# galatolofederico/clip-glass

Hardware: AMD Instinct MI355X
Metric: candidate latents scored/sec (GAN→CLIP fitness), StyleGAN2_ffhq_d pop=64 (higher is better)
Workload: dtype f16; 1 GPU; StyleGAN2_ffhq_d: StyleGAN2 config-f 1024px G+D + CLIP ViT-B/32, pop=64 per GPU, batch_size=4, n_obj=2; pop_per_gpu=64, global_pop=64, batch_size=4, parallelism=population-shard x1, device=AMD Radeon Graphics (gfx950:sramecc+:xnack-), 256 CUs, hbm_gib=288

## Files before the change

### clip_glass_amd/csrc/clip.cpp

```cpp
#include <math.h>
#include <string.h>

#include "engine.h"

extern "C" int glass_clip_geometry_supported(int32_t width, int32_t layers, int32_t heads, int32_t patch, int32_t res, int32_t embed) {
    char msg[256];
#define GEOM_REQ(cond, ...)                       \
    if (!(cond)) {                                \
        snprintf(msg, sizeof msg, __VA_ARGS__);   \
        glass_set_error(msg);                     \
        return GLASS_ERR_ARG;                     \
    }
    GEOM_REQ(width > 0 && layers > 0 && heads > 0 && patch > 0 && res > 0 && embed > 0,
             "unsupported CLIP geometry: width, layers, heads, patch, resolution and embed must be positive");
    GEOM_REQ(width % heads == 0 && width / heads == 64,
             "unsupported CLIP geometry: head dim must be 64 (width %d / heads %d)", width, heads);
    GEOM_REQ(res % patch == 0, "unsupported CLIP geometry: resolution %d is not a multiple of patch %d", res, patch);
    GEOM_REQ(patch <= 64 && res / patch <= 63,
             "unsupported CLIP geometry: patch %d / grid %d out of range (patch <= 64, at most 63 x 63 patches)", patch, res / patch);
    GEOM_REQ(layers <= 64 && width <= 4096 && embed <= 4096, "unsupported CLIP geometry: layers %d / width %d / embed %d out of range",
             layers, width, embed);
#undef GEOM_REQ
    return GLASS_OK;
}
int clip_patch_k(const glass_config& c) { return (3 * c.clip_patch * c.clip_patch + 63) / 64 * 64; }

extern "C" int glass_clip_preprocess_supported(int32_t gen_res, int32_t clip_res, int32_t clip_resize, int32_t clip_normalize) {
    if (clip_resize < 0 || clip_resize > 2) {
        glass_set_error("clip_resize must be 0 (point-sampled bilinear: the reference), 1 (antialiased bilinear) or 2 (antialiased bicubic), got " +
                        std::to_string(clip_resize));
        return GLASS_ERR_ARG;
    }
    if (clip_normalize < 0 || clip_normalize > 1) {
        glass_set_error("clip_normalize must be 0 (none: the reference) or 1 (CLIP mean / std), got " + std::to_string(clip_normalize));
        return GLASS_ERR_ARG;
    }
    if (clip_resize == 0 || gen_res == 0) return GLASS_OK;
    ResizeTaps t;
    std::string why;
    if (!build_resize_taps(gen_res, clip_res, clip_resize, t, why)) {
        glass_set_error(why);
        return GLASS_ERR_ARG;
    }
    return GLASS_OK;
}

static int load_clip_blocks(glass_engine* e, const char* prefix, int layers, int W, std::vector<ClipBlock>& out) {
    char nm[256];
    int rc;
    for (int i = 0; i < layers; ++i) {
        snprintf(nm, sizeof nm, "%s%d.", prefix, i);
        const std::string p = nm;
        ClipBlock b;
        GET(l1g, p + "ln_1.weight");
        GET(l1b, p + "ln_1.bias");
        GET(l2g, p + "ln_2.weight");
        GET(l2b, p + "ln_2.bias");
        GET(wq, p + "attn.in_proj_weight");
        GET(bq, p + "attn.in_proj_bias");
        GET(wo, p + "attn.out_proj.weight");
        GET(bo, p + "attn.out_proj.bias");
        GET(wf, p + "mlp.c_fc.weight");
        GET(bf, p + "mlp.c_fc.bias");
        GET(wp, p + "mlp.c_proj.weight");
        GET(bp, p + "mlp.c_proj.bias");
        REQUIRE(numel(wq) == (size_t)3 * W * W && numel(wo) == (size_t)W * W && numel(wf) == (size_t)4 * W * W &&
                    numel(wp) == (size_t)4 * W * W,
                GLASS_ERR_ARG, "bad CLIP block shapes: " + p);
        if ((rc = upload(e, &b.ln1_g, l1g->data))) return rc;
        if ((rc = upload(e, &b.ln1_b, l1b->data))) return rc;
        if ((rc = upload(e, &b.ln2_g, l2g->data))) return rc;
        if ((rc = upload(e, &b.ln2_b, l2b->data))) return rc;
        if ((rc = upload(e, &b.w_qkv, to_half(wq->data.data(), numel(wq))))) return rc;
        if ((rc = upload(e, &b.w_out, to_half(wo->data.data(), numel(wo))))) return rc;
        if ((rc = upload(e, &b.w_fc, to_half(wf->data.data(), numel(wf))))) return rc;
        if ((rc = upload(e, &b.w_proj, to_half(wp->data.data(), numel(wp))))) return rc;
        if ((rc = upload(e, &b.b_qkv, bq->data))) return rc;
        if ((rc = upload(e, &b.b_out, bo->data))) return rc;
        if ((rc = upload(e, &b.b_fc, bf->data))) return rc;
        if ((rc = upload(e, &b.b_proj, bp->data))) return rc;
        out.push_back(b);
    }
    return GLASS_OK;
}

int finalize_clip(glass_engine* e) {
    const glass_config& c = e->cfg;
    const int W = c.clip_width, ps = c.clip_patch, G = c.clip_res / ps, T = G * G + 1, E = c.clip_embed;
    const std::string v = "clip.visual.";
    GET(conv1, v + "conv1.weight");
    GET(cls, v + "class_embedding");
    GET(pos, v + "positional_embedding");
    GET(lg, v + "ln_pre.weight");
    GET(lb, v + "ln_pre.bias");
    GET(pg, v + "ln_post.weight");
    GET(pb, v + "ln_post.bias");
    GET(proj, v + "proj");
    REQUIRE(numel(conv1) == (size_t)W * 3 * ps * ps && numel(cls) == (size_t)W && numel(pos) == (size_t)T * W &&
                numel(proj) == (size_t)W * E,
            GLASS_ERR_ARG, "bad CLIP visual shapes");
    const int K = 3 * ps * ps, Kp = clip_patch_k(c);
    std::vector<_Float16> pw = to_half(conv1->data.data(), numel(conv1));
    if (Kp != K) {
        std::vector<_Float16> padded((size_t)W * Kp, (_Float16)0.f);
        for (int n = 0; n < W; ++n) std::copy(pw.begin() + (size_t)n * K, pw.begin() + (size_t)(n + 1) * K, padded.begin() + (size_t)n * Kp);
        pw.swap(padded);
    }
    int rc = upload(e, &e->c_patch_w, pw);
    if (rc) return rc;
    if ((rc = upload(e, &e->c_cls, cls->data))) return rc;
    if ((rc = upload(e, &e->c_pos, pos->data))) return rc;
    if ((rc = upload(e, &e->c_lnpre_g, lg->data))) return rc;
    if ((rc = upload(e, &e->c_lnpre_b, lb->data))) return rc;
    if ((rc = upload(e, &e->c_lnpost_g, pg->data))) return rc;
    if ((rc = upload(e, &e->c_lnpost_b, pb->data))) return rc;
    if ((rc = upload(e, &e->c_proj, proj->data))) return rc;
    int rc2 = load_clip_blocks(e, "clip.visual.transformer.resblocks.", c.clip_layers, W, e->cblk);
    if (rc2) return rc2;
    if (find(e, "clip.token_embedding.weight") != nullptr) {
        GET(tok, "clip.token_embedding.weight");
        GET(tpos, "clip.positional_embedding");
        GET(fg, "clip.ln_final.weight");
        GET(fb, "clip.ln_final.bias");
        GET(tp, "clip.text_projection");
        REQUIRE(tok->dims.size() == 2 && tpos->dims.size() == 2 && tpos->dims[1] == tok->dims[1], GLASS_ERR_ARG,
                "bad CLIP text embedding shapes");
        e->t_vocab = (int)tok->dims[0];
        e->t_width = (int)tok->dims[1];
        e->t_ctx = (int)tpos->dims[0];
        REQUIRE(e->t_width % 64 == 0 && numel(tp) == (size_t)e->t_width * E, GLASS_ERR_ARG, "bad CLIP text projection shape");
        int nl = 0;
        char nm2[256];
        for (;; ++nl) {
            snprintf(nm2, sizeof nm2, "clip.transformer.resblocks.%d.ln_1.weight", nl);
            if (!find(e, nm2)) break;
        }
        if ((rc = upload(e, &e->t_tok, tok->data))) return rc;
        if ((rc = upload(e, &e->t_pos, tpos->data))) return rc;
        if ((rc = upload(e, &e->t_lnf_g, fg->data))) return rc;
        if ((rc = upload(e, &e->t_lnf_b, fb->data))) return rc;
        if ((rc = upload(e, &e->t_proj, tp->data))) return rc;
        if ((rc = load_clip_blocks(e, "clip.transformer.resblocks.", nl, e->t_width, e->tblk))) return rc;
    }
    return GLASS_OK;
}

int finalize_preprocess(glass_engine* e) {
    const glass_config& c = e->cfg;
    if (c.clip_resize == 0 || e->R == 0) return GLASS_OK;
    ResizeTaps t;
    std::string why;
    REQUIRE(build_resize_taps(e->R, c.clip_res, c.clip_resize, t, why), GLASS_ERR_ARG, why);
    float* d_table = nullptr;
    int rc = upload(e, &d_table, t.table);
    if (rc) return rc;
    e->rz.table = d_table; e->rz.n4 = (int)(t.table.size() / 4); e->rz.ts = t.ts; e->rz.lds_bytes = t.lds_bytes;
    return GLASS_OK;
}

static void run_blocks(glass_engine* e, const std::vector<ClipBlock>& blk, int l0, int l1, float* x, half_t* ln16, half_t* qkv, half_t* att,
                       half_t* hid, int T, int seqs, int W, int heads, int causal, hipStream_t st, const char* pfx) {
    const int M = seqs * T;
    char buf[48];
    auto tag = [&](const char* op) -> const char* {
        if (!pfx) return nullptr;
        snprintf(buf, sizeof buf, "%s.%s", pfx, op);
        return buf;
    };
    auto gemm = [&](const GemmParams& g, const char* op) {
        if (pfx) run_gemm(e, g, tag(op));
        else if (!launch_gemm_tiled(g, st)) launch_gemm_direct(g, st);
    };
    auto layernorm = [&](const float* g, const float* b) {
        Prof pr(e, tag("layernorm"), 0, 6.0 * M * W);
        launch_layernorm(x, W, M, W, g, b, ln16, nullptr, st);
    };
    for (int li = l0; li < l1; ++li) {
        const ClipBlock& b = blk[li];
        layernorm(b.ln1_g, b.ln1_b);
        gemm(gemm_params(ln16, b.w_qkv, M, 3 * W, W, b.b_qkv, 0, qkv, nullptr, T), "qkv");
        {
            Prof pr(e, tag("attention"), 4.0 * seqs * heads * (double)T * T * 64, 8.0 * M * W);
            launch_attention(qkv, seqs, T, heads, 64, causal, att, st);
        }
        gemm(gemm_params(att, b.w_out, M, W, W, b.b_out, 2, nullptr, x, T), "attn_out");
        layernorm(b.ln2_g, b.ln2_b);
        gemm(gemm_params(ln16, b.w_fc, M, 4 * W, W, b.b_fc, 1, hid, nullptr, T), "mlp_fc");
        gemm(gemm_params(hid, b.w_proj, M, W, 4 * W, b.b_proj, 2, nullptr, x, T), "mlp_proj");
    }
}

void run_clip_embed(glass_engine* e, int P) {
    const glass_config& c = e->cfg;
    const int W = c.clip_width, G = c.clip_res / c.clip_patch, T = G * G + 1;
    run_gemm(e, gemm_params(e->d_patches, e->c_patch_w, P * G * G, W, clip_patch_k(c), nullptr, 3, nullptr, e->d_pe, G * G), "clip.patch_embed");
    Prof pr(e, "clip.embed_lnpre", 0, 8.0 * P * T * W);
    launch_embed_lnpre(e->d_pe, e->c_cls, e->c_pos, e->c_lnpre_g, e->c_lnpre_b, P, T, W, e->d_x, e->cur);
}
void run_clip_layers(glass_engine* e, int P, int l0, int l1) {
    const glass_config& c = e->cfg;
    const int G = c.clip_res / c.clip_patch;
    run_blocks(e, e->cblk, l0, std::min(l1, (int)e->cblk.size()), e->d_x, e->d_ln16, e->d_qkv, e->d_attn, e->d_hid, G * G + 1, P, c.clip_width, c.clip_heads, 0, e->cur, "clip");
}
void run_clip_head(glass_engine* e, int P) {
    const glass_config& c = e->cfg;
    const int W = c.clip_width, G = c.clip_res / c.clip_patch, T = G * G + 1;
    Prof pr(e, "clip.head", 2.0 * P * W * c.clip_embed, 4.0 * W * c.clip_embed);
    launch_layernorm(e->d_x, (long long)T * W, P, W, e->c_lnpost_g, e->c_lnpost_b, nullptr, e->d_cls, e->cur);
    launch_dense(e->d_cls, W, P, W, e->c_proj, c.clip_embed, nullptr, e->d_feat, c.clip_embed, 0, 0, nullptr, 0,
                 e->cur);
    launch_cosine(e->d_feat, e->d_target, P, c.clip_embed, e->d_sim, e->cur);
}
void run_clip(glass_engine* e, int P) {
    run_clip_embed(e, P);
    run_clip_layers(e, P, 0, (int)e->cblk.size());
    run_clip_head(e, P);
}

double clip_resize_bytes(const glass_engine* e, int B) {
    const glass_config& c = e->cfg;
    const double out = 2.0 * 3 * c.clip_res * c.clip_res;
    return B * ((c.clip_resize ? 4.0 * 3 * e->R * e->R : 16.0 * c.clip_res * c.clip_res * 3) + out);
}
void run_clip_resize(glass_engine* e, const float* y, int B, half_t* patches) {
    const glass_config& c = e->cfg;
    if (c.clip_resize == 0 && c.clip_normalize == 0)
        launch_resize_patches(y, B, e->R, c.clip_res, c.clip_patch, clip_patch_k(c), patches, e->cur);
    else
        launch_preprocess_patches(y, B, e->R, c.clip_res, c.clip_patch, clip_patch_k(c), c.clip_resize, c.clip_normalize, e->rz, patches, e->cur);
}

void text_work_free(glass_engine* e) {
    for (void* p : e->twork.owned) hipFree(p);
    e->twork = glass_engine::TextWork();
}

extern "C" int glass_engine_encode_text(glass_engine* e, const int32_t* tokens, int32_t n_texts, int32_t ctx, float* out_feat) {
    REQUIRE(e && tokens && out_feat && n_texts > 0, GLASS_ERR_ARG, "null argument");
    REQUIRE(e->finalized, GLASS_ERR_STATE, "finalize() first");
    REQUIRE(e->t_tok != nullptr, GLASS_ERR_STATE, "CLIP text tower weights were not loaded (clip.token_embedding.weight ...)");
    REQUIRE(ctx == e->t_ctx && ctx <= 128, GLASS_ERR_ARG, "context length does not match positional_embedding");
    GLASS_HIP(hipSetDevice(e->cfg.device));
    const int W = e->t_width, heads = W / 64, M = n_texts * ctx, E = e->cfg.clip_embed;
    std::vector<int> eot(n_texts);
    for (int n = 0; n < n_texts; ++n) {
        int best = 0;
        for (int t = 0; t < ctx; ++t) {
            const int v = tokens[(size_t)n * ctx + t];
            REQUIRE(v >= 0 && v < e->t_vocab, GLASS_ERR_ARG, "token id out of range");
            if (v > tokens[(size_t)n * ctx + best]) best = t;
        }
        eot[n] = best;
    }
    auto& tw = e->twork;
    hipError_t err = hipSuccess;
    if (tw.n_texts != n_texts) {
        text_work_free(e);
        if (err == hipSuccess) err = owned_alloc(tw.owned, &tw.d_tok, (size_t)M);
        if (err == hipSuccess) err = owned_alloc(tw.owned, &tw.d_rows, (size_t)n_texts);
        if (err == hipSuccess) err = owned_alloc(tw.owned, &tw.x, (size_t)M * W);
        if (err == hipSuccess) err = owned_alloc(tw.owned, &tw.cls, (size_t)n_texts * W);
        if (err == hipSuccess) err = owned_alloc(tw.owned, &tw.feat, (size_t)n_texts * E);
        if (err == hipSuccess) err = owned_alloc(tw.owned, &tw.ln16, (size_t)M * W);
        if (err == hipSuccess) err = owned_alloc(tw.owned, &tw.qkv, (size_t)M * 3 * W);
        if (err == hipSuccess) err = owned_alloc(tw.owned, &tw.att, (size_t)M * W);
        if (err == hipSuccess) err = owned_alloc(tw.owned, &tw.hid, (size_t)M * 4 * W);
        if (err != hipSuccess) {
            text_work_free(e);
            glass_set_error(std::string("encode_text: hipMalloc failed: ") + hipGetErrorString(err));
            return GLASS_ERR_NOMEM;
        }
        tw.n_texts = n_texts;
    }
    for (int n = 0; n < n_texts; ++n) eot[n] += n * ctx;
    hipStream_t st = e->stream;
    hipMemcpyAsync(tw.d_tok, tokens, (size_t)M * sizeof(int), hipMemcpyHostToDevice, st);
    hipMemcpyAsync(tw.d_rows, eot.data(), (size_t)n_texts * sizeof(int), hipMemcpyHostToDevice, st);
    launch_embed_text(tw.d_tok, e->t_tok, e->t_pos, M, ctx, W, tw.x, st);
    run_blocks(e, e->tblk, 0, (int)e->tblk.size(), tw.x, tw.ln16, tw.qkv, tw.att, tw.hid, ctx, n_texts, W, heads, 1, st, nullptr);
    launch_layernorm_rows(tw.x, tw.d_rows, n_texts, W, e->t_lnf_g, e->t_lnf_b, tw.cls, st);
    launch_dense(tw.cls, W, n_texts, W, e->t_proj, E, nullptr, tw.feat, E, 0, 0, nullptr, 0, st);
    err = hipMemcpyAsync(out_feat, tw.feat, (size_t)n_texts * E * sizeof(float), hipMemcpyDeviceToHost, st);
    if (err == hipSuccess) err = hipStreamSynchronize(st);
    if (err == hipSuccess) err = hipGetLastError();
    if (err != hipSuccess) {
        text_work_free(e);
        glass_set_error(std::string("encode_text failed: ") + hipGetErrorString(err));
        return GLASS_ERR_HIP;
    }
    return GLASS_OK;
}

extern "C" int glass_engine_encode_image(glass_engine* e, const float* images, int32_t n, float* out_feat) {
    REQUIRE(e && images && out_feat && n > 0, GLASS_ERR_ARG, "null argument");
    REQUIRE(e->finalized, GLASS_ERR_STATE, "finalize() first");
    REQUIRE(n <= e->cfg.max_pop, GLASS_ERR_ARG, "more images than max_pop");
    const glass_config& c = e->cfg;
    GLASS_HIP(hipSetDevice(c.device));
    const size_t elems = (size_t)n * 3 * c.clip_res * c.clip_res;
    float* d_img = nullptr;
    GLASS_HIP(hipMalloc(&d_img, elems * sizeof(float)));
    hipError_t err = hipMemcpyAsync(d_img, images, elems * sizeof(float), hipMemcpyHostToDevice, e->stream);
    e->cur = e->stream;
    launch_image_patches(d_img, n, c.clip_res, c.clip_patch, clip_patch_k(c), e->d_patches, e->stream);
    run_clip(e, n);
    if (err == hipSuccess)
        err = hipMemcpyAsync(out_feat, e->d_feat, (size_t)n * c.clip_embed * sizeof(float), hipMemcpyDeviceToHost, e->stream);
    if (err == hipSuccess) err = hipStreamSynchronize(e->stream);
    if (err == hipSuccess) err = hipGetLastError();
    hipFree(d_img);
    e->prof_events.clear();
    e->event_next = 0;
    if (err != hipSuccess) {
        glass_set_error(std::string("encode_image failed: ") + hipGetErrorString(err));
        return GLASS_ERR_HIP;
    }
    return GLASS_OK;
}
```

### clip_glass_amd/csrc/common.h

```cpp
#pragma once
#include <hip/hip_runtime.h>
#include <stdint.h>

#include <atomic>
#include <mutex>
#include <stdio.h>
#include <stdlib.h>

typedef _Float16 half_t;
typedef _Float16 h2 __attribute__((ext_vector_type(2)));
typedef _Float16 h4 __attribute__((ext_vector_type(4)));
typedef _Float16 h8 __attribute__((ext_vector_type(8)));
typedef float f4 __attribute__((ext_vector_type(4)));
typedef float f16x __attribute__((ext_vector_type(16)));

#define GLASS_SQRT2 1.41421356237309504880f

__device__ __forceinline__ f16x mfma32(h8 a, h8 b, f16x c) {
    return __builtin_amdgcn_mfma_f32_32x32x16_f16(a, b, c, 0, 0, 0);
}
__device__ __forceinline__ int mfma32_row(int reg, int lane) { return (reg & 3) + 8 * (reg >> 2) + 4 * (lane >> 5); }
__device__ __forceinline__ void philox4x32_10(uint32_t c[4], uint32_t k0, uint32_t k1) {
#pragma unroll
    for (int i = 0; i < 10; ++i) {
// ... 18 lines not shown
    const int my = oy >> 1, mx = ox >> 1;
    const float wy0 = (oy & 1) ? 0.25f : 0.75f, wx0 = (ox & 1) ? 0.25f : 0.75f;
    float s = 0.f;
    s += ((my >= 1 && mx >= 1) ? wy0 * wx0 : 0.f) * t[0];
    s += (my >= 1 ? wy0 * (1.f - wx0) : 0.f) * t[1];
    s += (mx >= 1 ? (1.f - wy0) * wx0 : 0.f) * t[2];
    s += (1.f - wy0) * (1.f - wx0) * t[3];
    return s;
}

struct DevOnce {
    std::atomic<bool> done[32] = {};
    static int dev() {
        int d = 0;
        if (hipGetDevice(&d) != hipSuccess || d < 0 || d >= 32) return -1;
        return d;
    }
    bool first() const {
        const int d = dev();
        return d < 0 || !done[d].load(std::memory_order_acquire);
    }
    void set() {
        const int d = dev();
        if (d >= 0) done[d].store(true, std::memory_order_release);
    }
    template <class F> void run(F&& setup) {
        if (first()) {
            setup();
            set();
        }
    }
};
struct GlassDevProps { int cus, lds_optin; };
inline GlassDevProps glass_dev_props() {
    static std::atomic<int> cus[32] = {}, lds[32] = {};
    int d = 0;
    if (hipGetDevice(&d) != hipSuccess || d < 0 || d >= 32) d = 0;
    if (!cus[d].load()) {
        hipDeviceProp_t prop;
        if (hipGetDeviceProperties(&prop, d) == hipSuccess) {
            lds[d].store((int)prop.sharedMemPerBlockOptin > 0 ? (int)prop.sharedMemPerBlockOptin : (int)prop.sharedMemPerBlock);
            cus[d].store(prop.multiProcessorCount);
        }
    }
    return GlassDevProps{cus[d].load() > 0 ? cus[d].load() : 256, lds[d].load() > 0 ? lds[d].load() : 64 * 1024};
}
inline int glass_cu_count() { return glass_dev_props().cus; }
inline bool glass_lds_fits(int bytes) {
    const GlassDevProps dp = glass_dev_props();
    if (bytes <= dp.lds_optin) return true;
    static std::mutex mu;
    static int seen_dev[16], seen_bytes[16], n_seen = 0;
    int d = 0;
    (void)hipGetDevice(&d);
    std::lock_guard<std::mutex> lk(mu);
    for (int i = 0; i < n_seen; ++i)
        if (seen_dev[i] == d && seen_bytes[i] == bytes) return false;
    if (n_seen == 16) return false;
    seen_dev[n_seen] = d;
    seen_bytes[n_seen++] = bytes;
    if (n_seen == 16) fprintf(stderr, "libglass: further LDS refusals are not reported\n");
    fprintf(stderr, "libglass: device %d offers %d B of opt-in LDS per workgroup; a kernel family that needs %d B is refused and its "
                    "layers fall back to a slower kernel (expected on gfx950: 163840 B)\n", d, dp.lds_optin, bytes);
    return false;
}

#define GLASS_NOMINAL_POP 64

__device__ __forceinline__ float lrelu_sqrt2(float v) { return (v > 0.f ? v : 0.2f * v) * GLASS_SQRT2; }
struct ActK { float k1, k2; };
__device__ __forceinline__ ActK act_consts(int act, float s) {
    return ActK{(act == 1 ? GLASS_SQRT2 : 1.f) * s, (act == 1 ? 0.2f * GLASS_SQRT2 : act == 2 ? 0.f : 1.f) * s};
}
__device__ __forceinline__ f4 act_apply(f4 v, ActK k) { return __builtin_elementwise_max(v * k.k1, v * k.k2); }

struct ConvParams {
    const half_t* x;
    long long x_bstride;
    int B, H, W, Cin;
    int Hc, Wc;
    int KS, stride, pad;
    const half_t* w;
    const half_t* w_up;
    long long w_bstride;
    int Neff, Cout;
    int up;
    int Ho, Wo;
    const float* sn;
    int sn_stride;
    const half_t* sn16;
    const half_t* pre_shift16;
    const float* pre_shift;
    int in_up;
    const float* dscale;
    int ds_stride;
    const float* noise;
    float noise_strength;
    int batch_size;
    const float* bias;
    const float* shift;
    int act;
    const half_t* res;
    int res_cs;
    int res_up;
    float out_scale;
    const float* rgb_y;
    const float* rgb_w;
    const float* rgb_b;
    half_t* rgb_x_out;
    half_t* rgb_xs_out;
    const float* trgb_w;
    const float* trgb_b;
    const float* trgb_sn;
    int trgb_sn_stride;
    const float* trgb_smax;
    int trgb_smax_stride;
    const float* trgb_yprev;
    float* trgb_yout;
    float* rgb_tanh_out;
    float* trgb_part;
    const half_t* trgb_tab;
    half_t* xs_out;
    const half_t* post_scale16;
    int post_stride;
    const half_t* skip_x;
    const half_t* skip_w;
    int dry_run;
    int x_planar32;
    int x_planar8;
    int y_planar8;
    int row_walk;
    half_t* y;
    float* y32;
};

struct GemmParams {
    const half_t* a;
    const half_t* w;
    int M, N, K;
    const float* bias;
    int mode;
    half_t* out16;
    float* out32;
    int ldo;
    int kpt;
    long long w_tap_stride;
    int batch;
    long long a_bs, w_bs, o_bs;
    int cand_rows;
    int cand_batch;
    int g_on, g_h, g_w, g_hc, g_wc, g_stride, g_pad, g_ks, g_cin;
    long long g_xbs;
    int ld;
};
```

### clip_glass_amd/csrc/engine.cpp

```cpp
#include "engine.h"

#include <math.h>
#include <string.h>

#include <stdlib.h>

static thread_local std::string g_err;
void glass_set_error(const std::string& s) { g_err = s; }
extern "C" const char* glass_last_error(void) { return g_err.c_str(); }
extern "C" const char* glass_version(void) { return "clip-glass-amd 0.1 (gfx950)"; }

void glass_pack_conv(const float* W, int cout, int cin, int ks, int cin_pad, std::vector<_Float16>& out) {
    const float coef = 1.0f / sqrtf((float)cin * ks * ks);
    out.assign((size_t)ks * ks * cout * cin_pad, (_Float16)0.f);
    for (int o = 0; o < cout; ++o)
        for (int i = 0; i < cin; ++i)
            for (int t = 0; t < ks * ks; ++t)
                out[((size_t)t * cout + o) * cin_pad + i] = (_Float16)(W[((size_t)o * cin + i) * ks * ks + t] * coef);
}

int glass_fold_upconv(const float* W, int cout, int cin, std::vector<_Float16>& out) {
    const float coef = 1.0f / sqrtf((float)cin * 9.f);
    const float f1[4] = {1.f, 3.f, 3.f, 1.f};
    float F[4][4];
// ... 324 lines not shown
        DBlock d;
        d.cin = chD(i);
        d.cout = chD(i + 1);
        d.res = e->R >> i;
        snprintf(nm, sizeof nm, "D.conv_blocks.%d", i);
        const std::string p = nm;
        GET(W0, p + ".conv_block.0.layer.weight");
        GET(B0, p + ".conv_block.0.bias");
        GET(W1, p + ".conv_block.1.layer.weight");
        GET(B1, p + ".conv_block.1.bias");
        GET(WS, p + ".projection.weight");
        REQUIRE(numel(W0) == (size_t)d.cin * d.cin * 9 && numel(W1) == (size_t)d.cout * d.cin * 9 &&
                    numel(WS) == (size_t)d.cout * d.cin && numel(B0) == (size_t)d.cin && numel(B1) == (size_t)d.cout,
                GLASS_ERR_ARG, "bad D block shape: " + p);
        std::vector<_Float16> pk;
        glass_pack_conv(W0->data.data(), d.cin, d.cin, 3, d.cin, pk);
        int rc = upload(e, &d.w0, pk);
        if (rc) return rc;
        glass_pack_conv(W1->data.data(), d.cout, d.cin, 3, d.cin, pk);
        rc = upload(e, &d.w1, pk);
        if (rc) return rc;
        glass_pack_conv(WS->data.data(), d.cout, d.cin, 1, d.cin, pk);
        rc = upload(e, &d.wskip, pk);
        if (rc) return rc;
        rc = upload(e, &d.b0, B0->data);
        if (rc) return rc;
        rc = upload(e, &d.b1, B1->data);
        if (rc) return rc;
        e->dblk.push_back(d);
    }
    const int CL = chD(n - 1);
    snprintf(nm, sizeof nm, "D.conv_blocks.%d.1.conv_block.0", n - 1);
    const std::string p = nm;
    GET(WF, p + ".layer.weight");
    GET(BF, p + ".bias");
    REQUIRE(numel(WF) == (size_t)CL * (CL + 1) * 9 && numel(BF) == (size_t)CL, GLASS_ERR_ARG, "bad D final conv shape");
    e->d_final_cpad = ((CL + 1 + 15) / 16) * 16;
    std::vector<_Float16> pk;
    glass_pack_conv(WF->data.data(), CL, CL + 1, 3, e->d_final_cpad, pk);
    int rc = upload(e, &e->d_final_w, pk);
    if (rc) return rc;
    rc = upload(e, &e->d_final_b, BF->data);
    if (rc) return rc;
    GET(W0, "D.dense.0.layer.weight");
    GET(B0, "D.dense.0.bias");
    GET(W1, "D.dense.1.layer.weight");
    GET(B1, "D.dense.1.bias");
    REQUIRE(numel(W0) == (size_t)CL * CL * 16 && numel(B0) == (size_t)CL && numel(W1) == (size_t)CL && numel(B1) == 1,
            GLASS_ERR_ARG, "bad D dense shape");
    std::vector<_Float16> d0((size_t)CL * CL * 16);
    const float coef0 = 1.0f / sqrtf((float)CL * 16.f);
    for (int o = 0; o < CL; ++o)
        for (int ch = 0; ch < CL; ++ch)
            for (int px = 0; px < 16; ++px)
                d0[(size_t)o * CL * 16 + (size_t)px * CL + ch] = (_Float16)(W0->data[(size_t)o * CL * 16 + ch * 16 + px] * coef0);
    rc = upload(e, &e->d_dense0_w, d0);
    if (rc) return rc;
    rc = upload(e, &e->d_dense0_b, B0->data);
    if (rc) return rc;
    rc = upload(e, &e->d_dense1_wt, transposed(W1->data.data(), 1, CL, 1.0f / sqrtf((float)CL)));
    if (rc) return rc;
    return upload(e, &e->d_dense1_b, B1->data);
}

static int alloc_buffers(glass_engine* e) {
    const glass_config& c = e->cfg;
    const int P = c.max_pop, L = c.latent_size, CH = e->chunk;
    int rc;
    if ((rc = dev_alloc(e, &e->d_z, (size_t)P * L))) return rc;
    if ((rc = dev_alloc(e, &e->d_w0, (size_t)P * L))) return rc;
    if ((rc = dev_alloc(e, &e->d_w1, (size_t)P * L))) return rc;
    if ((rc = dev_alloc(e, &e->d_s, (size_t)P * e->S_total))) return rc;
    if ((rc = dev_alloc(e, &e->d_s16, (size_t)P * e->S_total))) return rc;
    if ((rc = dev_alloc(e, &e->d_smax, (size_t)P * e->n_style))) return rc;
    if ((rc = dev_alloc(e, &e->d_trgb_tab, (size_t)P * 32 * 512))) return rc;
    {
        size_t part = 0;
        for (int b = 0; b < c.n_blocks; ++b)
            if (c.channels[b] > 128 && c.channels[b] % 128 == 0 && c.channels[b] <= 512)
                part = std::max(part, (size_t)(c.channels[b] / 128) * (size_t)P * 3 * ((size_t)4 << b) * ((size_t)4 << b));
        if (part && (rc = dev_alloc(e, &e->d_trgb_part, part))) return rc;
    }
    if (e->cfg.generator != GLASS_GEN_BIGGAN_DEEP && e->cfg.n_blocks > 0) {
        int cmax = 16;
        for (int i = 0; i < e->cfg.n_blocks; ++i) cmax = std::max(cmax, (int)e->cfg.channels[i]);
        e->cap_a = 256LL * 9 * cmax;
        e->cap_c = 256LL * 4 * cmax;
        if ((rc = dev_alloc(e, &e->ws_a, (size_t)(e->cap_a * P)))) return rc;
        if ((rc = dev_alloc(e, &e->ws_c, (size_t)(e->cap_c * P)))) return rc;
        if (e->cfg.use_discriminator) {
            if ((rc = dev_alloc(e, &e->ws_a2, (size_t)(e->cap_a * P)))) return rc;
            if ((rc = dev_alloc(e, &e->ws_c2, (size_t)(e->cap_c * P)))) return rc;
        }
    } else if (e->cfg.generator == GLASS_GEN_BIGGAN_DEEP) {
        const int cmax = 4 * e->cfg.bg_ch;
        e->cap_a = 256LL * 9 * cmax;
        e->cap_c = 256LL * 4 * cmax;
        if ((rc = dev_alloc(e, &e->ws_a, (size_t)(e->cap_a * P)))) return rc;
        if ((rc = dev_alloc(e, &e->ws_c, (size_t)(e->cap_c * P)))) return rc;
    }
    if ((rc = dev_alloc(e, &e->d_epsrow, (size_t)P * e->n_style))) return rc;
    if ((rc = dev_alloc(e, &e->d_dscale, (size_t)P * e->D_total))) return rc;
    for (auto& g : e->gconv) {
        const bool fused_ok = g.up && g.cin % 32 == 0 && g.cout % 32 == 0 && g.res_in >= 16;
        const bool tiled_ok = !g.up && g.cin % 32 == 0 && g.cout % 32 == 0 && g.res_in % 32 == 0;
        g.welems = 9LL * g.cin * g.cout;
        g.premod = (fused_ok || tiled_ok) && g.welems * 2 <= (500LL << 10);
        if (g.premod && (rc = dev_alloc(e, &g.wm, (size_t)P * g.welems))) return rc;
    }
    if (c.noise_mode != 0) {
        const int n_mb = P / c.batch_size;
        for (auto& g : e->gconv) {
            float* p;
            if ((rc = dev_alloc(e, &p, (size_t)n_mb * g.res_out * g.res_out))) return rc;
            e->d_noise.push_back(p);
        }
    }
    size_t maxact = 0;
    for (int b = 0; b < c.n_blocks; ++b) {
        const size_t res = 4u << b;
        size_t ch = c.channels[b];
        if (b > 0) ch = std::max<size_t>(ch, c.channels[b - 1]);
        maxact = std::max(maxact, (res + 1) * (res + 1) * ch);
    }
    if (c.n_blocks > 0) maxact = std::max(maxact, (size_t)16 * (c.channels[0] + 16));
    e->act_elems = maxact * CH;
    for (int i = 0; i < 8 && c.n_blocks > 0; ++i)
        if (i >= 6 || c.use_discriminator)
            if ((rc = dev_alloc(e, &e->act[i], e->act_elems))) return rc;
    for (int i = 0; i < 4; ++i)
        if ((rc = dev_alloc(e, &e->ybuf[i], (size_t)CH * 3 * e->R * e->R))) return rc;
    if (c.n_blocks > 0) {
        e->n_low = 0;
        while (e->n_low < c.n_blocks && (4 << e->n_low) <= e->low_res) ++e->n_low;
        if (e->n_low < 1) e->n_low = 1;
        const size_t rl = 4u << (e->n_low - 1);
        size_t cmax = 16;
        for (int b = 0; b < e->n_low; ++b) cmax = std::max<size_t>(cmax, c.channels[b]);
        if (e->n_low < c.n_blocks) cmax = std::max<size_t>(cmax, c.channels[e->n_low]);
        const size_t low_elems = (size_t)P * (rl + 1) * (rl + 1) * (cmax + 16);
        const int n_lowbuf = c.use_discriminator ? 6 : 2;
        for (int i = 0; i < n_lowbuf; ++i)
            if ((rc = dev_alloc(e, &e->low[i], low_elems))) return rc;
        for (int i = 0; i < 2; ++i)
            if ((rc = dev_alloc(e, &e->ylow[i], (size_t)P * 3 * rl * rl))) return rc;
    }
    if ((rc = dev_alloc(e, &e->d_img, (size_t)CH * 3 * e->R * e->R))) return rc;
    const int W = c.clip_width, ps = c.clip_patch, G = c.clip_res / ps, T = G * G + 1;
    const size_t Kp = (size_t)clip_patch_k(c);
    if ((rc = dev_alloc(e, &e->d_patches, (size_t)P * G * G * Kp))) return rc;
    if (Kp != (size_t)3 * ps * ps) GLASS_HIP(hipMemset(e->d_patches, 0, (size_t)P * G * G * Kp * sizeof(half_t)));
    if ((rc = dev_alloc(e, &e->d_pe, (size_t)P * G * G * W))) return rc;
    if ((rc = dev_alloc(e, &e->d_x, (size_t)P * T * W))) return rc;
    if ((rc = dev_alloc(e, &e->d_ln16, (size_t)P * T * W))) return rc;
    if ((rc = dev_alloc(e, &e->d_qkv, (size_t)P * T * 3 * W))) return rc;
    if ((rc = dev_alloc(e, &e->d_attn, (size_t)P * T * W))) return rc;
    if ((rc = dev_alloc(e, &e->d_hid, (size_t)P * T * 4 * W))) return rc;
    if ((rc = dev_alloc(e, &e->d_cls, (size_t)P * W))) return rc;
    if ((rc = dev_alloc(e, &e->d_feat, (size_t)P * c.clip_embed))) return rc;
    if ((rc = dev_alloc(e, &e->d_sim, (size_t)P))) return rc;
    if ((rc = dev_alloc(e, &e->d_dis, (size_t)P))) return rc;
    if ((rc = dev_alloc(e, &e->d_F, (size_t)P * 2))) return rc;
    if ((rc = dev_alloc(e, &e->d_target, (size_t)c.clip_embed))) return rc;
    if (c.use_discriminator && c.n_blocks > 0) {
        if ((rc = dev_alloc(e, &e->d_dfin, (size_t)P * 16 * c.channels[0]))) return rc;
        if ((rc = dev_alloc(e, &e->d_dh, (size_t)P * c.channels[0]))) return rc;
        if ((rc = dev_alloc(e, &e->d_dh_part, (size_t)16 * P * c.channels[0]))) return rc;
    }
    {
        std::vector<DenseDesc> dd;
        for (auto& g : e->gconv) {
            DenseDesc q;
            q.x = e->d_s + g.style_off; q.ldx = e->S_total; q.K = g.cin; q.wt = g.wsq; q.N = g.cout; q.bias = nullptr;
            q.out = e->d_dscale + g.ds_off; q.ldo = e->D_total; q.eps_row = e->d_epsrow + g.style_idx; q.eps_stride = e->n_style;
            dd.push_back(q);
            e->demod_max_n = std::max(e->demod_max_n, g.cout);
        }
        DenseDesc* dptr = nullptr;
        if ((rc = upload(e, &dptr, dd))) return rc;
        e->d_demod_desc = dptr;
    }
    GLASS_HIP(hipMemset(e->d_dis, 0, (size_t)P * sizeof(float)));
    e->h_pinned_bytes = std::max((size_t)P * L, (size_t)P * (c.clip_embed + 8)) * sizeof(float);
    GLASS_HIP(hipHostMalloc((void**)&e->h_pinned, e->h_pinned_bytes, hipHostMallocDefault));
    return GLASS_OK;
}

extern "C" int glass_engine_finalize(glass_engine* e) {
    REQUIRE(e, GLASS_ERR_ARG, "null engine");
    REQUIRE(!e->finalized, GLASS_ERR_STATE, "engine already finalized");
    GLASS_HIP(hipSetDevice(e->cfg.device));
    int rc = GLASS_OK;
    if (e->cfg.n_blocks > 0) {
        if ((rc = finalize_generator(e))) return rc;
        if (e->cfg.use_discriminator && (rc = finalize_discriminator(e))) return rc;
    }
    if (e->cfg.generator == GLASS_GEN_BIGGAN_DEEP && (rc = glass_biggan_finalize(e))) return rc;
    if ((rc = finalize_gpt2(e))) return rc;
    if ((rc = finalize_clip(e))) return rc;
    if ((rc = finalize_preprocess(e))) return rc;
    if ((rc = alloc_buffers(e))) return rc;
    e->host.clear();
    e->finalized = true;
    return GLASS_OK;
}

extern "C" int glass_engine_set_target(glass_engine* e, const float* feat, int32_t n) {
    REQUIRE(e && feat, GLASS_ERR_ARG, "null argument");
    REQUIRE(e->finalized, GLASS_ERR_STATE, "finalize() first");
    REQUIRE(n == e->cfg.clip_embed, GLASS_ERR_ARG, "target feature length != clip_embed");
    GLASS_HIP(hipSetDevice(e->cfg.device));
    GLASS_HIP(hipMemcpy(e->d_target, feat, (size_t)n * sizeof(float), hipMemcpyHostToDevice));
    e->has_target = true;
    return GLASS_OK;
}

void collect_profile(glass_engine* e) {
    std::map<std::string, glass_prof_row> rows;
    std::vector<std::string> order;
    for (auto& pe : e->prof_events) {
        float ms = 0.f;
        hipEventElapsedTime(&ms, pe.e0, pe.e1);
        auto it = rows.find(pe.name);
        if (it == rows.end()) {
            glass_prof_row r;
            memset(&r, 0, sizeof r);
            strncpy(r.name, pe.name.c_str(), sizeof(r.name) - 1);
            it = rows.emplace(pe.name, r).first;
            order.push_back(pe.name);
        }
        it->second.launches += 1;
        it->second.total_ms += ms;
        it->second.flops += pe.flops;
        it->second.bytes += pe.bytes;
    }
    e->prof_rows.clear();
    for (auto& n : order) e->prof_rows.push_back(rows[n]);
    e->prof_events.clear();
    e->event_next = 0;
}

void run_conv(glass_engine* e, const ConvParams& p, const char* tag, double flops, double bytes) {
    if (!(p.out_scale > 0.f)) {
        if (e->launch_error.empty()) e->launch_error = std::string("out_scale must be positive: ") + tag;
        return;
    }
    Prof pr(e, tag, flops, bytes);
    const char* k = p.up ? launch_upconv_fused(p, e->cur) : nullptr;
    if (p.rgb_tanh_out) {
        k = launch_conv_tiled(p, e->cur);
        if (!k && e->launch_error.empty()) e->launch_error = std::string("no kernel writes the planar tanh output of layer ") + tag;
        if (!k) k = "(refused)";
        pr.ran(tag, k);
        return;
    }
    if (!k) k = launch_conv_stream(p, e->cur);
    if (!k) k = launch_conv_glds(p, e->cur);
    if (!k) k = launch_conv_tiled(p, e->cur);
    if (!k) {
        const bool second = e->cur == e->stream_d && e->ws_a2;
        k = launch_conv_gemm(p, second ? e->ws_a2 : e->ws_a, e->cap_a, second ? e->ws_c2 : e->ws_c, e->cap_c, e->cur);
    }
    if (!k) k = launch_conv_direct(p, e->cur);
    if (!k) {
        if (e->launch_error.empty()) e->launch_error = std::string("no kernel accepts layer ") + tag;
        k = "(refused)";
    }
    pr.ran(tag, k);
}
void run_gemm(glass_engine* e, const GemmParams& p, const char* tag) {
    Prof pr(e, tag, 2.0 * p.M * p.N * p.K, 2.0 * ((double)p.M * p.K + (double)p.N * p.K + (double)p.M * p.N));
    const char* k = launch_gemm_tiled(p, e->cur);
    if (!k) k = launch_gemm_direct(p, e->cur);
    pr.ran(tag, k);
}

ConvParams conv_defaults() {
    ConvParams p;
    memset(&p, 0, sizeof p);
    p.out_scale = 1.f;
    p.batch_size = 1;
    p.stride = 1;
    return p;
}

GemmParams gemm_params(const half_t* a, const half_t* w, int M, int N, int K, const float* bias, int mode, half_t* out16, float* out32,
                       int cand_rows) {
    GemmParams g;
    memset(&g, 0, sizeof g);
    g.a = a; g.w = w; g.M = M; g.N = N; g.K = K; g.bias = bias; g.mode = mode;
    g.out16 = out16; g.out32 = out32; g.ldo = N; g.cand_rows = cand_rows;
    return g;
}

static int upload_noise(glass_engine* e, int P, int generation, int first_mb, const glass_noise* noise) {
    const glass_config& c = e->cfg;
    const int n_mb = P / c.batch_size;
    if (c.noise_mode == 1) {
        for (size_t l = 0; l < e->gconv.size(); ++l) {
            const int hw = e->gconv[l].res_out * e->gconv[l].res_out;
            Prof pr(e, "noise", 0, (double)n_mb * hw * 4);
            launch_noise(e->d_noise[l], n_mb, hw, (uint32_t)l, (uint32_t)first_mb, (uint32_t)generation, c.noise_seed,
                         e->cur);
        }
    } else if (c.noise_mode == 2) {
        REQUIRE(noise && noise->planes, GLASS_ERR_ARG, "noise_mode 2 requires caller-provided noise planes");
        REQUIRE(noise->n_layers == (int)e->gconv.size() && noise->n_minibatches >= n_mb, GLASS_ERR_ARG,
                "noise: wrong number of layers / minibatches");
        for (int m = 0; m < n_mb; ++m)
            for (size_t l = 0; l < e->gconv.size(); ++l) {
                const size_t hw = (size_t)e->gconv[l].res_out * e->gconv[l].res_out;
                const float* src = noise->planes[(size_t)m * noise->n_layers + l];
                REQUIRE(src, GLASS_ERR_ARG, "noise: null plane");
                GLASS_HIP(hipMemcpyAsync(e->d_noise[l] + (size_t)m * hw, src, hw * sizeof(float), hipMemcpyHostToDevice,
                                         e->cur));
            }
        GLASS_HIP(hipStreamSynchronize(e->cur));
    }
    return GLASS_OK;
}

static void run_styles(glass_engine* e, int P) {
    const glass_config& c = e->cfg;
    const int L = c.latent_size;
    {
        Prof pr(e, "mapping", 2.0 * P * L * L * c.mapping_layers, 4.0 * L * L * c.mapping_layers);
        if (c.mapping_layers < 1 ||
            !launch_mapping_fused(e->d_z, e->d_w0, P, L, 1e-8f, e->map_wt.data(), e->map_b.data(), c.mapping_layers, e->cur)) {
            launch_pixelnorm(e->d_z, e->d_w0, P, L, 1e-8f, e->cur);
            float *a = e->d_w0, *b = e->d_w1;
            for (int i = 0; i < c.mapping_layers; ++i) {
                if (L % 64 == 0 && L <= 768) launch_dense_splitk(a, L, P, L, e->map_wt[i], L, e->map_b[i], b, L, 1, e->cur);
                else launch_dense(a, L, P, L, e->map_wt[i], L, e->map_b[i], b, L, 0, 1, nullptr, 0, e->cur);
                std::swap(a, b);
            }
            if (a != e->d_w0)
                hipMemcpyAsync(e->d_w0, a, (size_t)P * L * sizeof(float), hipMemcpyDeviceToDevice, e->cur);
        }
    }
    {
        Prof pr(e, "styles", 2.0 * P * L * e->S_total, 4.0 * L * e->S_total);
        launch_dense(e->d_w0, L, P, L, e->style_wt, e->S_total, e->style_b, e->d_s, e->S_total, 0, 0, nullptr, 0,
                     e->cur);
        launch_style_norm(e->d_s, e->S_total, P, e->n_style, e->d_style_off, e->d_style_len, e->d_smax, e->d_epsrow,
                          1e-8f, e->cur);
        launch_bg_to_half(e->d_s, e->d_s16, (long long)P * e->S_total, e->cur);
    }
    {
        Prof pr(e, "demod", 0, 0);
        launch_dense_multi((const DenseDesc*)e->d_demod_desc, (int)e->gconv.size(), e->demod_max_n, P, 1, 2, e->cur);
    }
    {
        Prof pr(e, "premod_weights", 0, 0);
        for (auto& g : e->gconv)
            if (g.premod)
                launch_modulate_weights(g.up ? g.w_up : g.w, g.welems, g.cin, g.cout, e->d_s + g.style_off, e->S_total,
                                        e->d_dscale + g.ds_off, e->D_total, P, g.wm, e->cur);
    }
}

static void run_g_blocks(glass_engine* e, int c0, int B, int b_lo, int b_hi, const half_t* x, long long xbs,
                         half_t* const pp[2], const float* yprev, float* const yb[2], const half_t** x_out,
                         const float** y_out) {
    const glass_config& c = e->cfg;
    char tag[48];
    int gi = b_lo == 0 ? 0 : 1 + 2 * (b_lo - 1);
    int yi = 0;
    for (int b = b_lo; b < b_hi; ++b) {
        const int nl = b == 0 ? 1 : 2;
        bool rgb_done = false, pre_styled = false, x_planar = false;
        for (int l = 0; l < nl; ++l, ++gi) {
            const GConv& g = e->gconv[gi];
            ConvParams p = conv_defaults();
            p.x = x;
            p.x_bstride = xbs;
            p.B = B;
            p.H = p.W = g.res_in;
            p.Cin = g.cin;
            p.Hc = p.Wc = g.res_in;
            p.KS = 3;
            p.pad = 1;
            p.w = g.w;
            p.w_up = g.w_up;
            p.Cout = g.cout;
            p.up = g.up;
            p.Neff = g.up ? 4 * g.cout : g.cout;
            p.Ho = p.Wo = g.res_out;
            p.sn = e->d_s + (size_t)c0 * e->S_total + g.style_off;
            p.sn16 = e->d_s16 + (size_t)c0 * e->S_total + g.style_off;
            p.sn_stride = e->S_total;
            p.dscale = e->d_dscale + (size_t)c0 * e->D_total + g.ds_off;
            p.ds_stride = e->D_total;
            if (c.noise_mode != 0) {
                p.noise = e->d_noise[g.noise_idx] + (size_t)(c0 / c.batch_size) * g.res_out * g.res_out;
                p.noise_strength = g.noise_strength;
            }
            p.batch_size = c.batch_size;
            p.bias = g.bias;
            p.act = 1;
            if (g.premod) {
                p.sn = nullptr;
                p.sn16 = nullptr;
                p.dscale = nullptr;
                p.w_bstride = g.welems;
                if (g.up) { p.w_up = g.wm + (size_t)c0 * g.welems; p.w = nullptr; }
                else p.w = g.wm + (size_t)c0 * g.welems;
            }
            if (pre_styled) { p.sn = nullptr; p.sn16 = nullptr; pre_styled = false; }
            if (x_planar) { p.x_planar8 = 1; x_planar = false; }
            if (g.up && l == 0 && nl == 2 && !e->gconv[gi + 1].premod && !e->gconv[gi + 1].up) {
                ConvParams dq = p;
                dq.dry_run = 1;
                dq.y = pp[0];
                if (launch_upconv_fused(dq, e->cur)) {
                    const GConv& g2 = e->gconv[gi + 1];
                    p.post_scale16 = e->d_s16 + (size_t)c0 * e->S_total + g2.style_off;
                    p.post_stride = e->S_total;
                    pre_styled = true;
                }
            }
            half_t* out = pp[(x == pp[0]) ? 1 : 0];
            p.y = out;
            if (g.up && l == 0 && nl == 2 && !e->gconv[gi + 1].up && (pre_styled || e->gconv[gi + 1].premod) &&
                conv_wreg_supported(e->gconv[gi + 1].cin, e->gconv[gi + 1].cout, g.res_out, g.res_out)) {
                ConvParams dq = p;
// ... 507 lines not shown
```

### clip_glass_amd/csrc/engine.h

```cpp
#pragma once
#include <hip/hip_runtime.h>

#include <algorithm>
#include <map>
#include <string>
#include <vector>

#include "../../include/glass.h"
#include "common.h"
#include "kernels.h"

void glass_set_error(const std::string& s);
#define GLASS_HIP(call)                                                                        \
    do {                                                                                       \
        hipError_t _e = (call);                                                                \
        if (_e != hipSuccess) {                                                                \
            glass_set_error(std::string(#call) + " failed: " + hipGetErrorString(_e) + " at " + \
                            __FILE__ + ":" + std::to_string(__LINE__));                        \
            return GLASS_ERR_HIP;                                                              \
        }                                                                                      \
    } while (0)

struct HostTensor {
    std::vector<int64_t> dims;
    std::vector<float> data;
};

struct GConv {
    int cin, cout, res_in, res_out, up;
    int style_idx, style_off, ds_off, noise_idx;
    half_t* w = nullptr;
    half_t* w_up = nullptr;
    half_t* wm = nullptr;
    long long welems = 0;
    bool premod = false;
    float* wsq = nullptr;
    float* bias = nullptr;
    float noise_strength = 0.f;
};
struct GRgb {
    int cin, res, style_idx, style_off;
    float* w = nullptr;
    float* bias = nullptr;
};
struct DBlock {
    int cin, cout, res;
    half_t *w0 = nullptr, *w1 = nullptr, *wskip = nullptr;
    float *b0 = nullptr, *b1 = nullptr;
};
struct ClipBlock {
    float *ln1_g, *ln1_b, *ln2_g, *ln2_b;
    half_t *w_qkv, *w_out, *w_fc, *w_proj;
    float *b_qkv, *b_out, *b_fc, *b_proj;
};

struct BgBlock {
    int cin, cout, mid, up, res_in;
    int bn_off[4];
    half_t* w[4] = {nullptr, nullptr, nullptr, nullptr};
    float* b3 = nullptr;
};
struct BgState {
    int R = 0, Ctot = 0, zd = 0, nc = 0, c0 = 0;
    float *et = nullptr, *genz_wt = nullptr, *genz_b = nullptr;
    float *bn_wt = nullptr, *bn_bias = nullptr, *bn_inv_std = nullptr, *bn_mean = nullptr, *bn_prebias = nullptr;
    std::vector<BgBlock> blocks;
    int attn_before = -1, attn_C = 0, attn_res = 0;
    half_t *attn_w_tpg = nullptr, *attn_w_o = nullptr;
    int final_bn_off = 0, rgb_cpad = 32;
    half_t* rgb_w = nullptr;
    float* rgb_b = nullptr;
    half_t* tab16 = nullptr;
    float *cond = nullptr, *tab = nullptr, *h32 = nullptr, *a_S = nullptr;
    half_t *x[2] = {nullptr, nullptr}, *t1 = nullptr, *t2 = nullptr, *t3 = nullptr;
    half_t *a_T = nullptr, *a_theta = nullptr, *a_phi = nullptr, *a_gT = nullptr, *a_P = nullptr, *a_O = nullptr;
};
int glass_biggan_finalize(glass_engine* e);
int glass_biggan_prepare(glass_engine* e, int P);
int glass_biggan_chunk(glass_engine* e, int c0, int B, float* y);

struct ProfEvent {
    std::string name;
    double flops, bytes;
    hipEvent_t e0, e1;
};

struct glass_engine {
    glass_config cfg;
    int R = 0;
    int n_style = 0;
    int S_total = 0, D_total = 0;
    int chunk = 0;
    bool finalized = false, has_target = false;
    hipStream_t stream = nullptr, stream_d = nullptr, cur = nullptr;
    bool overlap = false, clip_overlap = false;
    std::vector<hipEvent_t> ev_g, ev_d;
    hipEvent_t ev0 = nullptr, ev1 = nullptr, ev_noise = nullptr;
    float last_ms = 0.f;
    int last_P = 0;
    std::string launch_error;

    std::map<std::string, HostTensor> host;
    std::vector<void*> allocs;

    std::vector<float*> map_wt, map_b;
    float *style_wt = nullptr, *style_b = nullptr;
    int *d_style_off = nullptr, *d_style_len = nullptr;
    std::vector<int> style_off, style_len;
    half_t* g_const = nullptr;
    void* d_demod_desc = nullptr;
    int demod_max_n = 0;
    std::vector<GConv> gconv;
    std::vector<GRgb> grgb;
    BgState bg;
    float *d_frgb_w = nullptr, *d_frgb_b = nullptr;
    std::vector<DBlock> dblk;
    half_t* d_final_w = nullptr;
    float* d_final_b = nullptr;
    int d_final_cpad = 0;
    half_t* d_dense0_w = nullptr;
    float *d_dense0_b = nullptr, *d_dense1_wt = nullptr, *d_dense1_b = nullptr;
    half_t* c_patch_w = nullptr;
    float *c_cls = nullptr, *c_pos = nullptr, *c_lnpre_g = nullptr, *c_lnpre_b = nullptr;
    float *c_lnpost_g = nullptr, *c_lnpost_b = nullptr, *c_proj = nullptr;
    std::vector<ClipBlock> cblk;
    ResizeTapsDev rz;
    struct Gpt2Block { float *ln1_g, *ln1_b, *ln2_g, *ln2_b, *w_qkv, *b_qkv, *w_o, *b_o, *w_fc, *b_fc, *w_pr, *b_pr; };
    std::vector<Gpt2Block> gblk;
    float *g_wte = nullptr, *g_wpe = nullptr, *g_lnf_g = nullptr, *g_lnf_b = nullptr;
    int g_vocab = 0, g_dim = 0, g_npos = 0;
    struct Gpt2Work {
        int P = 0, nctx = 0, length = 0;
        int *d_tok = nullptr, *d_gen = nullptr, *d_state = nullptr, *d_samp = nullptr;
        int sample = 0;
        float *x = nullptr, *ln = nullptr, *qkv = nullptr, *att = nullptr, *hid = nullptr, *last = nullptr, *logits = nullptr,
              *kc = nullptr, *vc = nullptr, *part = nullptr, *stats = nullptr, *pairs = nullptr, *pst = nullptr;
        size_t part_elems = 0;
        hipGraph_t graph = nullptr;
        hipGraphExec_t exec = nullptr;
        float last_ms = 0.f;
        std::vector<void*> owned;
    } gwork, gwork_alt;
    std::vector<ClipBlock> tblk;
    float *t_tok = nullptr, *t_pos = nullptr, *t_lnf_g = nullptr, *t_lnf_b = nullptr, *t_proj = nullptr;
    struct TextWork {
        int n_texts = 0;
        int *d_tok = nullptr, *d_rows = nullptr;
        float *x = nullptr, *cls = nullptr, *feat = nullptr;
        half_t *ln16 = nullptr, *qkv = nullptr, *att = nullptr, *hid = nullptr;
        std::vector<void*> owned;
    } twork;
    int t_width = 0, t_ctx = 0, t_vocab = 0;
    float* d_target = nullptr;

    half_t* d_s16 = nullptr;
    half_t* ws_a = nullptr;
    float* ws_c = nullptr;
    half_t* ws_a2 = nullptr;
    float* ws_c2 = nullptr;
    long long cap_a = 0, cap_c = 0;
    half_t* d_trgb_tab = nullptr;
    float* d_trgb_part = nullptr;
    float *d_z = nullptr, *d_w0 = nullptr, *d_w1 = nullptr, *d_s = nullptr, *d_smax = nullptr, *d_epsrow = nullptr,
          *d_dscale = nullptr;
    std::vector<float*> d_noise;
    half_t* act[8] = {nullptr, nullptr, nullptr, nullptr, nullptr, nullptr, nullptr, nullptr};
    half_t* low[6] = {nullptr, nullptr, nullptr, nullptr, nullptr, nullptr};
    float* ylow[2] = {nullptr, nullptr};
    int low_res = 32, n_low = 0;
    size_t act_elems = 0;
    float* ybuf[4] = {nullptr, nullptr, nullptr, nullptr};
    float* d_img = nullptr;
    half_t *d_patches = nullptr, *d_ln16 = nullptr, *d_qkv = nullptr, *d_attn = nullptr, *d_hid = nullptr;
    float *d_pe = nullptr, *d_x = nullptr, *d_cls = nullptr, *d_feat = nullptr, *d_sim = nullptr, *d_dis = nullptr,
          *d_F = nullptr, *d_dh = nullptr, *d_dh_part = nullptr;
    half_t* d_dfin = nullptr;
    float* h_pinned = nullptr;
    size_t h_pinned_bytes = 0;

    int bg_tap = -2;
    std::vector<float> bg_tap_data;
    int bg_tap_dims[4] = {0, 0, 0, 0};
    bool profiling = false;
    std::string prof_filter;
    std::map<std::string, std::string> tag_kernel;
    std::vector<ProfEvent> prof_events;
    std::vector<glass_prof_row> prof_rows;
    std::vector<hipEvent_t> event_pool;
    size_t event_next = 0;
};

#define REQUIRE(cond, code, msg)          \
    do {                                  \
        if (!(cond)) {                    \
            glass_set_error(msg);         \
            return code;                  \
        }                                 \
    } while (0)

template <typename T>
inline hipError_t owned_alloc(std::vector<void*>& owned, T** p, size_t n) {
    void* q = nullptr;
    const hipError_t err = hipMalloc(&q, n * sizeof(T));
    if (err != hipSuccess) return err;
    owned.push_back(q);
    *p = (T*)q;
    return hipSuccess;
}
template <typename T>
inline int dev_alloc(glass_engine* e, T** p, size_t n) {
    const hipError_t err = owned_alloc(e->allocs, p, std::max<size_t>(n, 1));
    if (err == hipSuccess) return GLASS_OK;
    glass_set_error(std::string("hipMalloc failed: ") + hipGetErrorString(err));
    return GLASS_ERR_NOMEM;
}
template <typename T>
inline int upload(glass_engine* e, T** p, const std::vector<T>& v) {
    int rc = dev_alloc(e, p, v.size());
    if (rc) return rc;
    GLASS_HIP(hipMemcpy(*p, v.data(), v.size() * sizeof(T), hipMemcpyHostToDevice));
    return GLASS_OK;
}

inline const HostTensor* find(glass_engine* e, const std::string& name) {
    auto it = e->host.find(name);
    return it == e->host.end() ? nullptr : &it->second;
}
#define GET(var, name)                                                            \
    const HostTensor* var = find(e, name);                                        \
    REQUIRE(var != nullptr, GLASS_ERR_STATE, std::string("missing tensor: ") + (name))

inline size_t numel(const HostTensor* t) {
    size_t n = 1;
    for (auto d : t->dims) n *= (size_t)d;
    return n;
}

struct Prof {
    glass_engine* e;
    bool on;
    ProfEvent pe;
    Prof(glass_engine* e_, const char* name, double flops, double bytes) : e(e_), on(name && e_->profiling) {
        if (on && !e->prof_filter.empty()) {
            auto it = e->tag_kernel.find(name);
            on = it != e->tag_kernel.end() && it->second.find(e->prof_filter) != std::string::npos;
        }
        if (!on) return;
        auto get = [&]() {
            if (e->event_next == e->event_pool.size()) {
                hipEvent_t ev;
                hipEventCreate(&ev);
                e->event_pool.push_back(ev);
            }
            return e->event_pool[e->event_next++];
        };
        pe.name = name;
        pe.flops = flops;
        pe.bytes = bytes;
        pe.e0 = get();
        pe.e1 = get();
        hipEventRecord(pe.e0, e->cur);
    }
    ~Prof() {
        if (!on) return;
        hipEventRecord(pe.e1, e->cur);
        e->prof_events.push_back(pe);
    }
    void ran(const char* tag, const char* k) {
        if (on) pe.name = std::string(tag) + "@" + k;
        if (e->profiling) e->tag_kernel[tag] = k;
    }
    void drop() { on = false; }
};

void collect_profile(glass_engine* e);
void run_conv(glass_engine* e, const ConvParams& p, const char* tag, double flops, double bytes);
void run_gemm(glass_engine* e, const GemmParams& p, const char* tag);
ConvParams conv_defaults();
GemmParams gemm_params(const half_t* a, const half_t* w, int M, int N, int K, const float* bias, int mode, half_t* out16, float* out32,
                       int cand_rows);

int clip_patch_k(const glass_config& c);
int finalize_clip(glass_engine* e);
int finalize_preprocess(glass_engine* e);
void text_work_free(glass_engine* e);
double clip_resize_bytes(const glass_engine* e, int B);
void run_clip_resize(glass_engine* e, const float* y, int B, half_t* patches);
void run_clip_embed(glass_engine* e, int P);
void run_clip_layers(glass_engine* e, int P, int l0, int l1);
void run_clip_head(glass_engine* e, int P);
void run_clip(glass_engine* e, int P);
#define GLASS_CLIP_SERIAL_LAYERS 1
std::vector<_Float16> to_half(const float* p, size_t n, float scale = 1.f);
std::vector<float> scaled(const float* p, size_t n, float scale);
std::vector<float> transposed(const float* W, int N, int K, float coef);


int finalize_gpt2(glass_engine* e);
void gpt2_work_free(glass_engine* e);

int glass_fold_upconv(const float* W, int cout, int cin, std::vector<_Float16>& out);
void glass_pack_conv(const float* W, int cout, int cin, int ks, int cin_pad, std::vector<_Float16>& out);
```

### clip_glass_amd/csrc/gemm_tiled.hip

```cpp
#include "common.h"
#include "kernels.h"
#include <stdlib.h>

#define GROWB 144

template <int BN, bool GATHER = false>
__global__ __launch_bounds__(256, 2) void gemm_tiled_kernel(GemmParams p) {
    if (p.batch > 1) {
        p.a += (long long)blockIdx.z * p.a_bs;
        p.w += (long long)blockIdx.z * p.w_bs;
        if (p.out16) p.out16 += (long long)blockIdx.z * p.o_bs;
        if (p.out32) p.out32 += (long long)blockIdx.z * p.o_bs;
    }
    constexpr int NJ = BN / 64;
    constexpr int NVA = 128 * 8, NVB = BN * 8;
    constexpr int NA = NVA / 256, NB = NVB / 256;
    __shared__ __attribute__((aligned(16))) char smem[(128 + BN) * GROWB];
    char* As = smem;
    char* Bs = smem + 128 * GROWB;
    const int t = threadIdx.x, lane = t & 63, wave = t >> 6;
    const int lr = lane & 31, kh = lane >> 5;
    const int wm = wave >> 1, wn = wave & 1;
    const int gy = p.N / BN, n_tiles = ((p.M + 127) >> 7) * gy;
    const int per_xcd = (n_tiles + 7) >> 3;
    const int tile = (blockIdx.x & 7) * per_xcd + (blockIdx.x >> 3);
    if (tile >= min(((int)(blockIdx.x & 7) + 1) * per_xcd, n_tiles)) return;
    const int m0 = (tile / gy) * 128, n0 = (tile % gy) * BN;
    const int part = t & 7;

    h8 ra[NA], rb[NB];
    long long gbase[GATHER ? NA : 1];
    int giy[GATHER ? NA : 1], gix[GATHER ? NA : 1], okm = 0;
    if (GATHER) {
#pragma unroll
        for (int k = 0; k < NA; ++k) {
            const int row = min(m0 + (t >> 3) + 32 * k, p.M - 1), hw = p.g_hc * p.g_wc;
            const int b = row / hw, rem = row - b * hw, oy = rem / p.g_wc, ox = rem - oy * p.g_wc;
            giy[k] = oy * p.g_stride - p.g_pad;
            gix[k] = ox * p.g_stride - p.g_pad;
            gbase[k] = (long long)b * p.g_xbs + ((long long)giy[k] * p.g_w + gix[k]) * p.g_cin + part * 8;
        }
    }
    auto load = [&](int k0) {
        const int kw = k0 + ((p.kpt && p.ld) ? (int)blockIdx.z * p.K : 0);
        if (GATHER) {
            const int tap = kw / p.g_cin, ci = kw - tap * p.g_cin, ty = tap / p.g_ks, tx = tap - ty * p.g_ks;
            const long long toff = ((long long)ty * p.g_w + tx) * p.g_cin + ci;
            okm = 0;
#pragma unroll
            for (int k = 0; k < NA; ++k) {
                const bool ok = (unsigned)(giy[k] + ty) < (unsigned)p.g_h && (unsigned)(gix[k] + tx) < (unsigned)p.g_w;
                ra[k] = *(const h8*)(p.a + (ok ? gbase[k] + toff : (long long)part * 8));
                okm |= (ok ? 1 : 0) << k;
            }
        } else {
#pragma unroll
        for (int k = 0; k < NA; ++k) {
            const int row = min(m0 + (t >> 3) + 32 * k, p.M - 1);
            ra[k] = *(const h8*)(p.a + (long long)row * (p.ld ? p.ld : p.K) + k0 + part * 8);
        }
        }
        const int rs = p.kpt ? p.kpt : (p.ld ? p.ld : p.K);
        const half_t* wk = p.kpt ? p.w + (long long)(kw / p.kpt) * p.w_tap_stride + (kw % p.kpt) : p.w + k0;
#pragma unroll
        for (int k = 0; k < NB; ++k) {
            const int row = (t >> 3) + 32 * k;
            rb[k] = *(const h8*)(wk + (long long)(n0 + row) * rs + part * 8);
        }
    };
    auto store = [&]() {
        const h8 zero = {0, 0, 0, 0, 0, 0, 0, 0};
#pragma unroll
        for (int k = 0; k < NA; ++k) *(h8*)(As + ((t >> 3) + 32 * k) * GROWB + part * 16) = (!GATHER || ((okm >> k) & 1)) ? ra[k] : zero;
#pragma unroll
        for (int k = 0; k < NB; ++k) *(h8*)(Bs + ((t >> 3) + 32 * k) * GROWB + part * 16) = rb[k];
    };

    f16x acc[2][NJ];
#pragma unroll
    for (int i = 0; i < 2; ++i)
#pragma unroll
        for (int j = 0; j < NJ; ++j)
#pragma unroll
            for (int q = 0; q < 16; ++q) acc[i][j][q] = 0.f;

    load(0);
    for (int k0 = 0; k0 < p.K; k0 += 64) {
        if (k0 > 0) __syncthreads();
        store();
        __syncthreads();
        if (k0 + 64 < p.K) load(k0 + 64);
#pragma unroll
        for (int kk = 0; kk < 4; ++kk) {
            h8 wf[NJ], xf[2];
#pragma unroll
            for (int j = 0; j < NJ; ++j)
                wf[j] = *(const h8*)(Bs + (wn * (BN / 2) + j * 32 + lr) * GROWB + kk * 32 + kh * 16);
#pragma unroll
            for (int i = 0; i < 2; ++i)
                xf[i] = *(const h8*)(As + (wm * 64 + i * 32 + lr) * GROWB + kk * 32 + kh * 16);
#pragma unroll
            for (int i = 0; i < 2; ++i)
#pragma unroll
                for (int j = 0; j < NJ; ++j) acc[i][j] = mfma32(wf[j], xf[i], acc[i][j]);
        }
    }
    f4 bq[NJ][4];
#pragma unroll
    for (int j = 0; j < NJ; ++j)
#pragma unroll
        for (int g = 0; g < 4; ++g) {
            bq[j][g] = f4{0.f, 0.f, 0.f, 0.f};
            if (p.bias) bq[j][g] = *(const f4*)(p.bias + n0 + wn * (BN / 2) + j * 32 + 8 * g + 4 * kh);
        }
#pragma unroll
    for (int i = 0; i < 2; ++i) {
        const int m = m0 + wm * 64 + i * 32 + lr;
        const int mc = min(m, p.M - 1);
        f4 rq[NJ][4];
        if (p.mode == 2) {
#pragma unroll
            for (int j = 0; j < NJ; ++j)
#pragma unroll
                for (int g = 0; g < 4; ++g)
                    rq[j][g] = *(const f4*)(p.out32 + (long long)mc * p.ldo + n0 + wn * (BN / 2) + j * 32 + 8 * g + 4 * kh);
        }
        if (m >= p.M) continue;
#pragma unroll
        for (int j = 0; j < NJ; ++j) {
#pragma unroll
            for (int g = 0; g < 4; ++g) {
                const int n = n0 + wn * (BN / 2) + j * 32 + 8 * g + 4 * kh;
                float v[4];
#pragma unroll
                for (int q = 0; q < 4; ++q) v[q] = acc[i][j][g * 4 + q] + bq[j][g][q];
                const long long oi = (long long)m * p.ldo + n;
                if (p.mode <= 1) {
                    h4 o;
#pragma unroll
                    for (int q = 0; q < 4; ++q)
                        o[q] = (half_t)(p.mode == 1 ? v[q] * __builtin_amdgcn_rcpf(1.f + __expf(-1.702f * v[q])) : v[q]);
                    *(h4*)(p.out16 + oi) = o;
                } else {
                    f4 o;
                    if (p.mode == 2) {
#pragma unroll
                        for (int q = 0; q < 4; ++q) o[q] = rq[j][g][q] + v[q];
                    } else {
#pragma unroll
                        for (int q = 0; q < 4; ++q) o[q] = p.mode == 4 ? lrelu_sqrt2(v[q]) : v[q];
                    }
                    *(f4*)(p.out32 + oi) = o;
                }
            }
        }
    }
}

const char* launch_gemm_tiled(const GemmParams& p, hipStream_t st) {
    if (p.K % 64 != 0 || p.ldo % 4 != 0 || (p.M < 64 && !p.kpt) || (p.kpt && p.kpt % 64 != 0)) return nullptr;
    const unsigned gx = (unsigned)((p.M + 127) / 128), gz = p.batch > 1 ? p.batch : 1;
    const long long gx_n = p.cand_rows ? ((long long)p.cand_rows * GLASS_NOMINAL_POP + 127) / 128 : gx;
    const long long gz_n = p.cand_batch ? GLASS_NOMINAL_POP : gz;
    const bool fills = gx_n * (p.N / 128) * gz_n >= 256;
    if (p.g_on && (!p.kpt || p.kpt != p.g_cin || p.g_cin % 64 != 0)) return nullptr;
    if (p.N % 128 == 0 && fills) {
        if (p.g_on) {
            hipLaunchKernelGGL((gemm_tiled_kernel<128, true>), dim3(8 * ((gx * (p.N / 128) + 7) / 8), 1, gz), dim3(256), 0, st, p);
            return "gemm_tiled_kernel<128,true>";
        }
        hipLaunchKernelGGL(gemm_tiled_kernel<128>, dim3(8 * ((gx * (p.N / 128) + 7) / 8), 1, gz), dim3(256), 0, st, p);
        return "gemm_tiled_kernel<128>";
    }
    if (p.N % 64 == 0) {
        if (p.g_on) {
            hipLaunchKernelGGL((gemm_tiled_kernel<64, true>), dim3(8 * ((gx * (p.N / 64) + 7) / 8), 1, gz), dim3(256), 0, st, p);
            return "gemm_tiled_kernel<64,true>";
        }
        hipLaunchKernelGGL(gemm_tiled_kernel<64>, dim3(8 * ((gx * (p.N / 64) + 7) / 8), 1, gz), dim3(256), 0, st, p);
        return "gemm_tiled_kernel<64>";
    }
    return nullptr;
}
```

### clip_glass_amd/csrc/kernels.h

```cpp
#pragma once
#include "common.h"

#include <string>
#include <vector>

const char* launch_conv_direct(const ConvParams& p, hipStream_t st);
const char* launch_gemm_direct(const GemmParams& p, hipStream_t st);
const char* launch_conv_tiled(const ConvParams& p, hipStream_t st);
const char* launch_gemm_tiled(const GemmParams& p, hipStream_t st);
const char* launch_conv_stream(const ConvParams& p, hipStream_t st);
const char* launch_conv_gemm(const ConvParams& p, half_t* ws_a, long long cap_a, float* ws_c, long long cap_c, hipStream_t st);
bool conv_stream_applies(const ConvParams& p);
const char* launch_conv_glds(const ConvParams& p, hipStream_t st);
const char* launch_conv_wreg(const ConvParams& p, hipStream_t st);
bool conv_wreg_supported(int Cin, int Cout, int H, int W);
const char* launch_conv_s2(const ConvParams& p, hipStream_t st, bool force = false);
const char* launch_conv_down(const half_t* h, const half_t* xs, const half_t* w1, const half_t* ws, const float* b1, half_t* y,
                             int B, int R, int Cin, int Cout, hipStream_t st);
bool conv_down_supported(int R, int Cin, int Cout);
const char* launch_dblock0(const float* rgb_y, const float* rgb_w, const float* rgb_b, const half_t* w0, const float* b0, const half_t* w1,
                           const half_t* ws, const float* b1, half_t* y, int B, int R, int Cin, int Cout, hipStream_t st, int y_planar8 = 0);
bool dblock0_supported(int R, int Cin, int Cout);
const char* launch_upconv_fused(const ConvParams& p, hipStream_t st);

void launch_pixelnorm(const float* z, float* out, int P, int L, float eps, hipStream_t st);
void launch_dense01_finish(const float* part, int S, long long slab, const float* bias0, const float* w1, const float* b1, float* out, int P, int N,
                           hipStream_t st);
void launch_dense_splitk(const float* x, int ldx, int P, int K, const float* wt, int N, const float* bias, float* out, int ldo,
                         int mode, hipStream_t st);
void launch_dense(const float* x, int ldx, int P, int K, const float* wt, int N, const float* bias,
                  float* out, int ldo, int in_sq, int mode, const float* eps_row, int eps_stride,
                  hipStream_t st);
bool launch_mapping_fused(const float* z, float* out, int P, int L, float eps, const float* const* wt, const float* const* b, int n_layers,
                          hipStream_t st);
struct DenseDesc {
    const float* x; int ldx; int K; const float* wt; int N; const float* bias; float* out; int ldo;
    const float* eps_row; int eps_stride;
};
void launch_dense_multi(const DenseDesc* d_desc, int n_desc, int max_N, int P, int in_sq, int mode, hipStream_t st);
void launch_style_norm(float* s, int ld, int P, int n_layers, const int* d_off, const int* d_len,
                       float* smax, float* eps_row, float eps, hipStream_t st);
void launch_modulate_weights(const half_t* w, long long elems, int Cin, int Cout, const float* sn, int sn_stride,
                              const float* dscale, int ds_stride, int P, half_t* wm, hipStream_t st);
void launch_noise(float* out, int n_mb, int hw, uint32_t layer, uint32_t mb0, uint32_t generation,
                  uint64_t seed, hipStream_t st);

void launch_trgb_tables(const float* wrgb, const float* sn, int sn_stride, const float* smax, int smax_stride, int B, int NT,
                        half_t* tab, hipStream_t st);
void launch_trgb_finish(const float* part, int ntn, int B, int R, const float* bias, const float* yprev, float* yout, hipStream_t st);
bool launch_torgb(const half_t* x, int B, int H, int W, int C, const float* wrgb, const float* bias,
                  const float* sn, int sn_stride, const float* smax, int smax_stride,
                  const float* yprev, float* yout, hipStream_t st);
void launch_finalize_image(const float* y, float* img, long long n, hipStream_t st);
void launch_resize_patches(const float* y, int B, int R, int clip_res, int ps, int ld, half_t* patches,
                           hipStream_t st);
#define GLASS_RESIZE_MAX_TAPS 32
#define PREPROCESS_TY 8
#define PREPROCESS_RB 8
#define PREPROCESS_MAX_R 1024
struct ResizeTaps {
    std::vector<int> start, count;
    std::vector<float> taps;
    std::vector<float> table;
    int max_count = 0, nr = 0, ts = 0;
    size_t lds_bytes = 0;
};
struct ResizeTapsDev {
    const float* table = nullptr;
    int n4 = 0, ts = 0;
    size_t lds_bytes = 0;
};
bool build_resize_taps(int R, int S, int mode, ResizeTaps& t, std::string& why);
void launch_preprocess_patches(const float* y, int B, int R, int clip_res, int ps, int ld, int resize_mode, int normalize,
                               const ResizeTapsDev& t, half_t* patches, hipStream_t st);
void launch_fromrgb(const float* y, int B, int R, int Cout, const float* w, const float* bias,
                    half_t* out, hipStream_t st);
void launch_blur_pad2(const half_t* x, int B, int H, int W, int C, half_t* out, hipStream_t st, int planar32 = 0);
bool blur_pad2_planar32_ok(int C);
void launch_blur_down(const half_t* x, int B, int H, int W, int C, half_t* out, hipStream_t st);
void launch_mbstd(const half_t* x, int B, int hw, int C, int Cpad, int batch_size, int group, float eps,
                  half_t* out, hipStream_t st);

void launch_embed_lnpre(const float* patch_emb, const float* cls, const float* pos, const float* g,
                        const float* b, int P, int T, int D, float* x, hipStream_t st);
void launch_embed_text(const int* tokens, const float* tok_emb, const float* pos, int n_rows, int ctx, int D, float* x,
                       hipStream_t st);
void launch_layernorm(const float* x, long long row_stride, int M, int D, const float* g, const float* b,
                      half_t* out16, float* out32, hipStream_t st);
void launch_layernorm_rows(const float* x, const int* rows, int M, int D, const float* g, const float* b, float* out32, hipStream_t st);
void launch_attention(const half_t* qkv, int n_img, int L, int heads, int hd, int causal, half_t* out,
                      hipStream_t st);
void launch_cosine(const float* feat, const float* target, int P, int D, float* sim, hipStream_t st);
void launch_assemble_F(const float* sim, const float* dis, int P, int n_obj, float* F, hipStream_t st);

void launch_bg_cond(const float* x, int P, int L, int zd, int nc, const float* et, float* cond, hipStream_t st);
void launch_bg_bn_tables(float* tab, int P, int C, const float* inv_std, const float* mean, const float* prebias,
                         hipStream_t st);
void launch_bg_to_half(const float* x, half_t* y, long long n, hipStream_t st);
void launch_bg_attn_split(const half_t* T, int B, int H, int W, int c8, int c2, half_t* theta, half_t* phi, half_t* gT,
                          hipStream_t st);
void launch_bg_softmax(const float* S, long long rows, int n, half_t* Pm, hipStream_t st);
void launch_bg_rgb_tanh(const half_t* x, int B, long long hw, int C, float* y, hipStream_t st);

struct BgTailParams {
    const half_t* h;
    const half_t* x0;
    const half_t* w3;
    const float* b3;
    const float* tab;
    int bnf_off, ctot;
    const half_t* rgb_w;
    int cpad;
    const float* rgb_b;
    float* y;
    int B, R;
};
bool bg_tail_supported(int R, int mid, int cout, int cin, int up, int cpad);
bool launch_bg_tail(const BgTailParams& p, hipStream_t st);
void launch_gpt2_embed(const int* tok, const float* wte, const float* wpe, int rows, int L, int pos0, int D, float* x,
                       hipStream_t st);
void launch_gemm_f32(const float* A, const float* W, const float* bias, float* out, int M, int N, int K, int lda, int ldo,
                     int mode, hipStream_t st, float* part = nullptr, size_t part_elems = 0, bool prefill = false);
bool gemm_f32_step_supported(int M, int K, int lda, bool ln_fused);
int launch_gemm_f32_step(const float* A, const float* W, const float* bias, float* out, int M, int N, int K, int lda, int ldo, int mode,
                         hipStream_t st, float* part, size_t part_elems, const float* stats, const float* lng, const float* lnb);
bool gpt2_head_supported(int M, int N, int K, int lda);
bool launch_gpt2_head_tail(const float* A, const float* W, int M, int N, int K, int lda, const float* stats_in, const float* lng, const float* lnb,
                           float* pairs, int* gen, int* state, const float* wte, const float* wpe, float* x, float* stats_out, hipStream_t st);
bool launch_gpt2_head(const float* A, const float* W, int M, int N, int K, int lda, const float* stats, const float* lng, const float* lnb,
                      float* logits, float* pairs, int* out, const int* step_dev, hipStream_t st);
void launch_gpt2_reduce(const float* part, int S, const float* bias, float* out, int M, int N, int ldo, int mode, hipStream_t st);
void launch_gpt2_finalize(const float* part, int S, const float* bias, float* x, int M, int D, float* stats, hipStream_t st);
#define GPT2_ATTENTION_LDS_MAX (160 * 1024)
size_t gpt2_attention_lds_bytes(int nd, int ns);
void launch_gpt2_attention(const float* qkv, float* kc, float* vc, int P, int nd, int past, int Tmax, int heads,
                           float* out, hipStream_t st, const int* past_dev = nullptr);
void launch_gpt2_attention_step(const float* qkv, const float* part, int S, const float* bias, float* kc, float* vc, int P, int Tmax, int heads,
                                float* out, hipStream_t st, const int* past_dev);
void launch_argmax(const float* logits, int rows, int N, int* out, hipStream_t st, const int* step_dev = nullptr, float* scratch = nullptr);
void launch_gpt2_embed_step(const int* gen, const int* state, int P, const float* wte, const float* wpe, int D, float* x, hipStream_t st,
                            float* stats = nullptr, bool partial_fmt = false);
bool gemm_f32_rowblk_supported(int M, int N, int K, int lda, bool ln_fused, bool stats_out);
bool launch_gemm_f32_rowblk(const float* A, const float* W, const float* bias, float* out, int M, int N, int K, int lda, int ldo, int mode,
                            hipStream_t st, const float* pst_in, int np_in, const float* lng, const float* lnb, float* pst_out);
void launch_gpt2_advance(int* state, hipStream_t st);
enum { GPT2_SP_SEED_LO, GPT2_SP_SEED_HI, GPT2_SP_GEN, GPT2_SP_ROW0, GPT2_SP_PURPOSE, GPT2_SP_TEMP, GPT2_SP_TOPK, GPT2_SP_STEP, GPT2_SP_WORDS };
#define GPT2_SAMPLE_TOPK_MAX 256
bool gpt2_sample_supported(int V);
void launch_gpt2_sample(const float* logits, int rows, int V, const int* sp, int* out, int* state, hipStream_t st);
bool launch_gpt2_head_sample(const float* A, const float* W, int M, int N, int K, int lda, const float* stats_in, const float* lng, const float* lnb,
                             float* logits, float* pairs, const int* sp, int* gen, int* state, bool tail, const float* wte, const float* wpe, float* x,
                             float* stats_out, hipStream_t st);
void launch_image_patches(const float* img, int n, int S, int ps, int ld, half_t* patches, hipStream_t st);
```

### clip_glass_amd/csrc/kernels_clip.hip

```cpp
#include "common.h"
#include "kernels.h"
#include <stdlib.h>

__device__ __forceinline__ float wsum(float v) {
#pragma unroll
    for (int o = 32; o > 0; o >>= 1) v += __shfl_xor(v, o);
    return v;
}

template <typename LoadF>
__device__ __forceinline__ void ln_row(LoadF load, int D, const float* g, const float* b, half_t* o16, float* o32) {
    const int lane = threadIdx.x & 63;
    if (D <= 1024) {
        float v[16];
#pragma unroll
        for (int k = 0; k < 16; ++k) v[k] = lane + 64 * k < D ? load(lane + 64 * k) : 0.f;
        float s = 0.f;
#pragma unroll
        for (int k = 0; k < 16; ++k) s += v[k];
        const float mean = wsum(s) / (float)D;
        float q = 0.f;
#pragma unroll
        for (int k = 0; k < 16; ++k) { const float d = lane + 64 * k < D ? v[k] - mean : 0.f; q += d * d; }
        const float rstd = rsqrtf(wsum(q) / (float)D + 1e-5f);
#pragma unroll
        for (int k = 0; k < 16; ++k) {
            const int i = lane + 64 * k;
            if (i < D) {
                const float o = (v[k] - mean) * rstd * g[i] + b[i];
                if (o16) o16[i] = (half_t)o;
                if (o32) o32[i] = o;
            }
        }
        return;
    }
    float s = 0.f;
    for (int i = lane; i < D; i += 64) s += load(i);
    const float mean = wsum(s) / (float)D;
    float q = 0.f;
    for (int i = lane; i < D; i += 64) { const float d = load(i) - mean; q += d * d; }
    const float rstd = rsqrtf(wsum(q) / (float)D + 1e-5f);
    for (int i = lane; i < D; i += 64) {
        const float v = (load(i) - mean) * rstd * g[i] + b[i];
        if (o16) o16[i] = (half_t)v;
        if (o32) o32[i] = v;
    }
}

__global__ __launch_bounds__(256) void embed_lnpre_kernel(const float* pe, const float* cls, const float* pos,
                                                          const float* g, const float* b, int P, int T, int D,
                                                          float* x) {
    const int row = blockIdx.x * 4 + (threadIdx.x >> 6);
    if (row >= P * T) return;
    const int p = row / T, t = row - p * T;
    const float* src = t == 0 ? cls : pe + ((long long)p * (T - 1) + (t - 1)) * D;
    const float* ps = pos + (long long)t * D;
    ln_row([&](int i) { return src[i] + ps[i]; }, D, g, b, nullptr, x + (long long)row * D);
}
void launch_embed_lnpre(const float* patch_emb, const float* cls, const float* pos, const float* g,
                        const float* b, int P, int T, int D, float* x, hipStream_t st) {
    hipLaunchKernelGGL(embed_lnpre_kernel, dim3((P * T + 3) / 4), dim3(256), 0, st, patch_emb, cls, pos, g, b, P,
                       T, D, x);
}

__global__ void embed_text_kernel(const int* tokens, const float* tok_emb, const float* pos, int ctx, int D, float* x) {
    const int row = blockIdx.x;
    const float* te = tok_emb + (long long)tokens[row] * D;
    const float* pe = pos + (long long)(row % ctx) * D;
    for (int i = threadIdx.x; i < D; i += blockDim.x) x[(long long)row * D + i] = te[i] + pe[i];
}
void launch_embed_text(const int* tokens, const float* tok_emb, const float* pos, int n_rows, int ctx, int D, float* x,
                       hipStream_t st) {
    hipLaunchKernelGGL(embed_text_kernel, dim3(n_rows), dim3(128), 0, st, tokens, tok_emb, pos, ctx, D, x);
}

__global__ __launch_bounds__(256) void layernorm_kernel(const float* x, long long row_stride, int M, int D,
                                                        const float* g, const float* b, half_t* o16, float* o32) {
    const int row = blockIdx.x * 4 + (threadIdx.x >> 6);
    if (row >= M) return;
    const float* xr = x + (long long)row * row_stride;
    ln_row([&](int i) { return xr[i]; }, D, g, b, o16 ? o16 + (long long)row * D : nullptr,
           o32 ? o32 + (long long)row * D : nullptr);
}
void launch_layernorm(const float* x, long long row_stride, int M, int D, const float* g, const float* b,
                      half_t* out16, float* out32, hipStream_t st) {
    hipLaunchKernelGGL(layernorm_kernel, dim3((M + 3) / 4), dim3(256), 0, st, x, row_stride, M, D, g, b, out16,
                       out32);
}

__global__ __launch_bounds__(256) void layernorm_rows_kernel(const float* x, const int* rows, int M, int D, const float* g, const float* b, float* o32) {
    const int m = blockIdx.x * 4 + (threadIdx.x >> 6);
    if (m >= M) return;
    const float* xr = x + (long long)rows[m] * D;
    ln_row([&](int i) { return xr[i]; }, D, g, b, nullptr, o32 + (long long)m * D);
}
void launch_layernorm_rows(const float* x, const int* rows, int M, int D, const float* g, const float* b, float* out32, hipStream_t st) {
    hipLaunchKernelGGL(layernorm_rows_kernel, dim3((M + 3) / 4), dim3(256), 0, st, x, rows, M, D, g, b, out32);
}

template <int NKB>
__global__ __launch_bounds__(256) void attention_mfma_kernel(const half_t* qkv, int L, int heads, int n_pairs, int causal,
                                                             half_t* out) {
    constexpr int PP = NKB == 2 ? 2 : 1;
    constexpr int WP = 4 / PP;
    constexpr int VROW = NKB * 64 + 16;
    __shared__ __attribute__((aligned(16))) char vts[PP][64 * VROW];
    const int t = threadIdx.x, lane = t & 63, wave = t >> 6, lr = lane & 31, kh = lane >> 5;
    const int pair = blockIdx.x * PP + wave / WP, qb = wave % WP;
    const int pc = min(pair, n_pairs - 1);
    const int img = pc / heads, h = pc - img * heads, D = heads * 64;
    const half_t* base = qkv + (long long)img * L * 3 * D + h * 64;
    const long long ts = 3LL * D;
    const int query = qb * 32 + lr;
    const bool qwave = qb < NKB;
    h8 qf[4], kf[NKB][4];
    if (qwave) {
        const half_t* qp = base + min(query, L - 1) * ts + kh * 8;
#pragma unroll
        for (int kk = 0; kk < 4; ++kk) qf[kk] = *(const h8*)(qp + kk * 16);
#pragma unroll
        for (int kb = 0; kb < NKB; ++kb) {
            const half_t* kp = base + min(kb * 32 + lr, L - 1) * ts + D + kh * 8;
#pragma unroll
            for (int kk = 0; kk < 4; ++kk) kf[kb][kk] = *(const h8*)(kp + kk * 16);
        }
    }
    constexpr int TP = 64 * WP;
    constexpr int NV = NKB * 32 * 8 / TP;
    const int pt = t % TP;
    h8 vv[NV];
#pragma unroll
    for (int u = 0; u < NV; ++u) {
        const int e = pt + TP * u, tok = e >> 3, d8 = e & 7;
        vv[u] = *(const h8*)(base + min(tok, L - 1) * ts + 2 * D + d8 * 8);
    }
    char* vt = vts[wave / WP];
#pragma unroll
    for (int u = 0; u < NV; ++u) {
        const int e = pt + TP * u, tok = e >> 3, d8 = e & 7;
        const int r = tok & 31, g = r >> 3;
        const int pos = ((tok >> 5) * 2 + (g >> 1)) * 16 + ((r >> 2) & 1) * 8 + (g & 1) * 4 + (r & 3);
#pragma unroll
        for (int j = 0; j < 8; ++j) *(half_t*)(vt + (d8 * 8 + j) * VROW + pos * 2) = tok < L ? vv[u][j] : (half_t)0.f;
    }
    f16x s[NKB];
    float inv = 0.f;
    if (qwave) {
#pragma unroll
        for (int kb = 0; kb < NKB; ++kb) {
#pragma unroll
            for (int r = 0; r < 16; ++r) s[kb][r] = 0.f;
#pragma unroll
            for (int kk = 0; kk < 4; ++kk) s[kb] = mfma32(kf[kb][kk], qf[kk], s[kb]);
        }
        float m = -INFINITY;
#pragma unroll
        for (int kb = 0; kb < NKB; ++kb)
#pragma unroll
            for (int r = 0; r < 16; ++r) {
                const int key = kb * 32 + (r & 3) + 8 * (r >> 2) + 4 * kh;
                float v = s[kb][r] * 0.125f;
                if (key >= L || (causal && key > query)) v = -INFINITY;
                s[kb][r] = v;
                m = fmaxf(m, v);
            }
        m = fmaxf(m, __shfl_xor(m, 32));
        float z = 0.f;
#pragma unroll
        for (int kb = 0; kb < NKB; ++kb)
#pragma unroll
            for (int r = 0; r < 16; ++r) {
                const float e2 = __expf(s[kb][r] - m);
                s[kb][r] = e2;
                z += e2;
            }
        z += __shfl_xor(z, 32);
        inv = 1.f / z;
    }
    __syncthreads();
    if (!qwave) return;
    f16x o[2], ol[2];
#pragma unroll
    for (int db = 0; db < 2; ++db)
#pragma unroll
        for (int r = 0; r < 16; ++r) { o[db][r] = 0.f; ol[db][r] = 0.f; }
#pragma unroll
    for (int ks = 0; ks < 2 * NKB; ++ks) {
        h8 ph, pl;
#pragma unroll
        for (int e = 0; e < 8; ++e) {
            const float pv = s[ks >> 1][(2 * (ks & 1) + (e >> 2)) * 4 + (e & 3)] * inv;
            ph[e] = (half_t)pv;
            pl[e] = (half_t)((pv - (float)ph[e]) * 2048.f);
        }
#pragma unroll
        for (int db = 0; db < 2; ++db) {
            const h8 vf = *(const h8*)(vt + (db * 32 + lr) * VROW + (ks * 16 + kh * 8) * 2);
            o[db] = mfma32(vf, ph, o[db]);
            ol[db] = mfma32(vf, pl, ol[db]);
        }
    }
    if (pair < n_pairs && query < L) {
        half_t* op = out + ((long long)img * L + query) * D + h * 64 + 4 * kh;
#pragma unroll
        for (int db = 0; db < 2; ++db)
#pragma unroll
            for (int g = 0; g < 4; ++g) {
                h4 w;
#pragma unroll
                for (int q = 0; q < 4; ++q) w[q] = (half_t)(o[db][g * 4 + q] + ol[db][g * 4 + q] * (1.f / 2048.f));
                *(h4*)(op + db * 32 + 8 * g) = w;
            }
    }
}

__global__ __launch_bounds__(256, 2) void attention_stream_kernel(const half_t* qkv, int L, int heads, int causal, half_t* out) {
    constexpr int ROW = 144, TILE = 64 * ROW;
    __shared__ __attribute__((aligned(16))) char kls[2][TILE];
    __shared__ __attribute__((aligned(16))) char vls[2][TILE];
    const int t = threadIdx.x, lane = t & 63, wave = t >> 6, lr = lane & 31, kh = lane >> 5;
    const int nqb = (L + 127) / 128;
    const int pair = blockIdx.x / nqb, qblk = blockIdx.x - pair * nqb;
    const int img = pair / heads, h = pair - img * heads, D = heads * 64;
    const half_t* base = qkv + (long long)img * L * 3 * D + h * 64;
    const long long ts = 3LL * D;
    const int q0 = qblk * 128 + wave * 32, query = q0 + lr;
// ... 9 lines not shown
#pragma unroll
        for (int u = 0; u < 2; ++u) {
            kr[u] = *(const h8*)(base + (long long)min(k0 + sk + 32 * u, L - 1) * ts + D + sd8 * 8);
            vr[u] = *(const h8*)(base + (long long)min(k0 + vtok + u, L - 1) * ts + 2 * D + vd8 * 8);
        }
    };
    auto stage_write = [&](int kt, int buf) {
        const int k0 = kt * 64;
#pragma unroll
        for (int u = 0; u < 2; ++u) *(h8*)(kls[buf] + (sk + 32 * u) * ROW + sd8 * 16) = kr[u];
        const bool ok0 = k0 + vtok < L, ok1 = k0 + vtok + 1 < L;
#pragma unroll
        for (int j = 0; j < 8; ++j) {
            h2 w;
            w[0] = ok0 ? vr[0][j] : (half_t)0.f;
            w[1] = ok1 ? vr[1][j] : (half_t)0.f;
            *(h2*)(vls[buf] + (vd8 * 8 + j) * ROW + vpos * 2) = w;
        }
    };
    h8 qf[4];
    {
        const half_t* qp = base + (long long)min(query, L - 1) * ts + kh * 8;
#pragma unroll
        for (int kk = 0; kk < 4; ++kk) qf[kk] = *(const h8*)(qp + kk * 16);
    }
    f16x o[2], ol[2];
#pragma unroll
    for (int db = 0; db < 2; ++db)
#pragma unroll
        for (int r = 0; r < 16; ++r) { o[db][r] = 0.f; ol[db][r] = 0.f; }
    float m = -INFINITY, z = 0.f;
    stage_load(0);
    stage_write(0, 0);
    __syncthreads();
    for (int kt = 0; kt < nkt; ++kt) {
        const int buf = kt & 1;
        const bool work = kt < wkt;
        f16x s[2];
        if (work) {
            const char* kl = kls[buf];
#pragma unroll
            for (int kb = 0; kb < 2; ++kb) {
#pragma unroll
                for (int r = 0; r < 16; ++r) s[kb][r] = 0.f;
#pragma unroll
                for (int kk = 0; kk < 4; ++kk) {
                    const h8 kf = *(const h8*)(kl + (kb * 32 + lr) * ROW + (kk * 16 + kh * 8) * 2);
                    s[kb] = mfma32(kf, qf[kk], s[kb]);
                }
            }
        }
        if (kt + 1 < nkt) stage_load(kt + 1);
        if (work) {
            const int k0 = kt * 64;
            float mt = -INFINITY;
#pragma unroll
            for (int kb = 0; kb < 2; ++kb)
#pragma unroll
                for (int r = 0; r < 16; ++r) {
                    const int key = k0 + kb * 32 + (r & 3) + 8 * (r >> 2) + 4 * kh;
                    float v = s[kb][r] * 0.125f;
                    if (key >= L || (causal && key > query)) v = -INFINITY;
                    s[kb][r] = v;
                    mt = fmaxf(mt, v);
                }
            mt = fmaxf(mt, __shfl_xor(mt, 32));
            const float mn = fmaxf(m, mt);
            const float alpha = __expf(m - mn);
            m = mn;
            float zt = 0.f;
#pragma unroll
            for (int kb = 0; kb < 2; ++kb)
#pragma unroll
                for (int r = 0; r < 16; ++r) {
                    const float e2 = __expf(s[kb][r] - mn);
                    s[kb][r] = e2;
                    zt += e2;
                }
            z = z * alpha + zt;
            if (__any(alpha != 1.f)) {
#pragma unroll
                for (int db = 0; db < 2; ++db)
#pragma unroll
                    for (int r = 0; r < 16; ++r) { o[db][r] *= alpha; ol[db][r] *= alpha; }
            }
            const char* vl = vls[buf];
#pragma unroll
            for (int ks = 0; ks < 4; ++ks) {
                h8 ph, pl;
#pragma unroll
                for (int e = 0; e < 8; ++e) {
                    const float pv = s[ks >> 1][(2 * (ks & 1) + (e >> 2)) * 4 + (e & 3)];
                    ph[e] = (half_t)pv;
                    pl[e] = (half_t)((pv - (float)ph[e]) * 2048.f);
                }
#pragma unroll
                for (int db = 0; db < 2; ++db) {
                    const h8 vf = *(const h8*)(vl + (db * 32 + lr) * ROW + (ks * 16 + kh * 8) * 2);
                    o[db] = mfma32(vf, ph, o[db]);
                    ol[db] = mfma32(vf, pl, ol[db]);
                }
            }
        }
        if (kt + 1 < nkt) stage_write(kt + 1, buf ^ 1);
        __syncthreads();
    }
    if (query < L) {
        z += __shfl_xor(z, 32);
        const float inv = 1.f / z;
        half_t* op = out + ((long long)img * L + query) * D + h * 64 + 4 * kh;
#pragma unroll
        for (int db = 0; db < 2; ++db)
#pragma unroll
            for (int g = 0; g < 4; ++g) {
                h4 w;
#pragma unroll
                for (int q = 0; q < 4; ++q) w[q] = (half_t)((o[db][g * 4 + q] + ol[db][g * 4 + q] * (1.f / 2048.f)) * inv);
                *(h4*)(op + db * 32 + 8 * g) = w;
            }
    }
}

void launch_attention(const half_t* qkv, int n_img, int L, int heads, int hd, int causal, half_t* out,
                      hipStream_t st) {
    (void)hd;
    if (L <= 64) {
        const int n_pairs = n_img * heads;
        hipLaunchKernelGGL(attention_mfma_kernel<2>, dim3((n_pairs + 1) / 2), dim3(256), 0, st, qkv, L, heads, n_pairs, causal, out);
        return;
    }
    if (L <= 96) {
        const int n_pairs = n_img * heads;
        hipLaunchKernelGGL(attention_mfma_kernel<3>, dim3(n_pairs), dim3(256), 0, st, qkv, L, heads, n_pairs, causal, out);
        return;
    }
    const int nqb = (L + 127) / 128;
    hipLaunchKernelGGL(attention_stream_kernel, dim3((unsigned)((long long)n_img * heads * nqb)), dim3(256), 0, st, qkv, L, heads, causal, out);
}

__global__ void cosine_kernel(const float* feat, const float* target, int D, float* sim) {
    const int p = blockIdx.x, lane = threadIdx.x;
    float xy = 0.f, xx = 0.f, yy = 0.f;
    for (int i = lane; i < D; i += 64) {
        const float a = feat[(long long)p * D + i], b = target[i];
        xy += a * b; xx += a * a; yy += b * b;
    }
    xy = wsum(xy); xx = wsum(xx); yy = wsum(yy);
    if (lane == 0) sim[p] = xy / fmaxf(sqrtf(xx) * sqrtf(yy), 1e-8f);
}
void launch_cosine(const float* feat, const float* target, int P, int D, float* sim, hipStream_t st) {
    hipLaunchKernelGGL(cosine_kernel, dim3(P), dim3(64), 0, st, feat, target, D, sim);
}

__global__ void assemble_F_kernel(const float* sim, const float* dis, int P, int n_obj, float* F) {
    const int p = blockIdx.x * blockDim.x + threadIdx.x;
    if (p >= P) return;
    F[(long long)p * n_obj] = -sim[p];
    if (n_obj == 2) F[(long long)p * n_obj + 1] = fmaxf(1.f - dis[p], 0.f);
}
void launch_assemble_F(const float* sim, const float* dis, int P, int n_obj, float* F, hipStream_t st) {
    hipLaunchKernelGGL(assemble_F_kernel, dim3((P + 63) / 64), dim3(64), 0, st, sim, dis, P, n_obj, F);
}

__global__ void image_patches_kernel(const float* img, int n, int S, int ps, int ld, half_t* patches) {
    const int G = S / ps;
    const long long idx = (long long)blockIdx.x * blockDim.x + threadIdx.x;
    if (idx >= (long long)n * 3 * S * S) return;
    const int X = (int)(idx % S), Y = (int)((idx / S) % S);
    const int c = (int)((idx / ((long long)S * S)) % 3), b = (int)(idx / ((long long)S * S * 3));
    const int gy = Y / ps, iy = Y - gy * ps, gx = X / ps, ix = X - gx * ps;
    const long long row = ((long long)b * G + gy) * G + gx;
    patches[row * ld + ((long long)c * ps + iy) * ps + ix] = (half_t)img[idx];
}
void launch_image_patches(const float* img, int n, int S, int ps, int ld, half_t* patches, hipStream_t st) {
    const long long total = (long long)n * 3 * S * S;
    hipLaunchKernelGGL(image_patches_kernel, dim3((unsigned)((total + 255) / 256)), dim3(256), 0, st, img, n, S, ps, ld, patches);
}
```

### clip_glass_amd/csrc/ops.hip

```cpp
#include <string.h>

#include <string>
#include <vector>

#include "../../include/glass_ops.h"
#include "engine.h"
#include "kernels.h"

namespace {
struct Dev {
    std::vector<void*> ptrs;
    ~Dev() {
        for (void* p : ptrs) hipFree(p);
    }
    template <typename T>
    T* alloc(size_t n) {
        void* q = nullptr;
        if (hipMalloc(&q, (n ? n : 1) * sizeof(T)) != hipSuccess) return nullptr;
        ptrs.push_back(q);
        return (T*)q;
    }
    half_t* up16(const float* src, size_t n) {
        if (!src) return nullptr;
        std::vector<_Float16> h(n);
// ... 203 lines not shown
    Dev dv;
    half_t* dx = dv.up16(x, (size_t)B * H * H * C);
    OPREQ(mode != 2 || blur_pad2_planar32_ok(C), "blur in 32-channel planes: C must be 32 x a power of two, <= 512");
    const int Ho = mode != 1 ? H + 1 : H / 2;
    half_t* dy = dv.alloc<half_t>((size_t)B * Ho * Ho * C);
    if (mode != 1) launch_blur_pad2(dx, B, H, H, C, dy, 0, mode == 2);
    else launch_blur_down(dx, B, H, H, C, dy, 0);
    int rc = finish();
    if (rc) return rc;
    return down16(out, dy, (size_t)B * Ho * Ho * C);
}

extern "C" int glass_op_dblock_down(int32_t device, int32_t B, int32_t R, int32_t Cin, int32_t Cout, const float* h,
                                    const float* x, const float* w1, const float* wskip, const float* b1, float* y) {
    OPREQ(h && x && w1 && wskip && b1 && y, "bad argument");
    GLASS_HIP(hipSetDevice(device));
    Dev dv;
    half_t* dh = dv.up16(h, (size_t)B * R * R * Cin);
    half_t* dx = dv.up16(x, (size_t)B * R * R * Cin);
    std::vector<_Float16> pk;
    glass_pack_conv(w1, Cout, Cin, 3, Cin, pk);
    half_t* dw1 = dv.up16v(pk);
    glass_pack_conv(wskip, Cout, Cin, 1, Cin, pk);
    half_t* dws = dv.up16v(pk);
    float* db = dv.up32(b1, Cout);
    const int Ro = R / 2;
    half_t* dxs = dv.alloc<half_t>((size_t)B * Ro * Ro * Cin);
    half_t* dy = dv.alloc<half_t>((size_t)B * Ro * Ro * Cout);
    OPREQ(conv_down_supported(R, Cin, Cout), "conv_down: unsupported shape");
    launch_blur_down(dx, B, R, R, Cin, dxs, 0);
    OPREQ(launch_conv_down(dh, dxs, dw1, dws, db, dy, B, R, Cin, Cout, 0) != nullptr, "conv_down: unsupported shape");
    int rc = finish();
    if (rc) return rc;
    return down16(y, dy, (size_t)B * Ro * Ro * Cout);
}

extern "C" int glass_op_dblock0(int32_t device, int32_t B, int32_t R, int32_t impl, const float* y, const float* frgb_w, const float* frgb_b,
                                const float* w0, const float* b0, const float* w1, const float* wskip, const float* b1, float* out) {
    OPREQ(y && frgb_w && frgb_b && w0 && b0 && w1 && wskip && b1 && out && B > 0 && R > 0, "bad argument");
    GLASS_HIP(hipSetDevice(device));
    Dev dv;
    const int Cin = 32, Cout = 64, Ro = R / 2;
    float* dy = dv.up32(y, (size_t)B * 3 * R * R);
    float* dfw = dv.up32(frgb_w, Cin * 3); float* dfb = dv.up32(frgb_b, Cin);
    std::vector<_Float16> pk;
    glass_pack_conv(w0, Cin, Cin, 3, Cin, pk);
    half_t* dw0 = dv.up16v(pk);
    glass_pack_conv(w1, Cout, Cin, 3, Cin, pk);
    half_t* dw1 = dv.up16v(pk);
    glass_pack_conv(wskip, Cout, Cin, 1, Cin, pk);
    half_t* dws = dv.up16v(pk);
    float* db0 = dv.up32(b0, Cin); float* db1 = dv.up32(b1, Cout);
    half_t* dout = dv.alloc<half_t>((size_t)B * Ro * Ro * Cout);
    OPREQ(dy && dw0 && dw1 && dws && dout, "device allocation failed");
    if (impl == 0 || impl == 2) {
        OPREQ(launch_dblock0(dy, dfw, dfb, dw0, db0, dw1, dws, db1, dout, B, R, Cin, Cout, 0, impl == 2) != nullptr, "dblock0: unsupported shape");
    } else {
        half_t* dh = dv.alloc<half_t>((size_t)B * R * R * Cin);
        half_t* dxs = dv.alloc<half_t>((size_t)B * Ro * Ro * Cin);
        OPREQ(dh && dxs, "device allocation failed");
        ConvParams p = conv_defaults();
        p.x = dh; p.x_bstride = (long long)R * R * Cin; p.B = B; p.H = p.W = R; p.Cin = Cin; p.Hc = p.Wc = R; p.KS = 3; p.pad = 1;
        p.w = dw0; p.Cout = p.Neff = Cin; p.Ho = p.Wo = R; p.bias = db0; p.act = 1; p.y = dh;
        p.rgb_y = dy; p.rgb_w = dfw; p.rgb_b = dfb; p.rgb_xs_out = dxs;
        OPREQ(launch_conv_stream(p, 0) != nullptr, "dblock0 (two-kernel form): conv_stream<fromrgb> does not take this shape");
        OPREQ(launch_conv_down(dh, dxs, dw1, dws, db1, dout, B, R, Cin, Cout, 0) != nullptr, "dblock0 (two-kernel form): conv_down does not take this shape");
    }
    int rc = finish();
    if (rc) return rc;
    return down16(out, dout, (size_t)B * Ro * Ro * Cout);
}

extern "C" int glass_op_fromrgb(int32_t device, int32_t B, int32_t R, int32_t Cout, const float* y, const float* w,
                                const float* bias, float* out) {
    OPREQ(y && w && bias && out && Cout % 8 == 0, "bad argument");
    GLASS_HIP(hipSetDevice(device));
    Dev dv;
    float* dy = dv.up32(y, (size_t)B * 3 * R * R); float* dw = dv.up32(w, Cout * 3); float* db = dv.up32(bias, Cout);
    half_t* dout = dv.alloc<half_t>((size_t)B * R * R * Cout);
    launch_fromrgb(dy, B, R, Cout, dw, db, dout, 0);
    int rc = finish();
    if (rc) return rc;
    return down16(out, dout, (size_t)B * R * R * Cout);
}

extern "C" int glass_op_mbstd(int32_t device, int32_t B, int32_t hw, int32_t C, int32_t Cpad, int32_t batch_size,
                              int32_t group, const float* x, float* out) {
    OPREQ(x && out && B % batch_size == 0 && batch_size % group == 0 && group <= 8, "bad argument");
    GLASS_HIP(hipSetDevice(device));
    Dev dv;
    half_t* dx = dv.up16(x, (size_t)B * hw * C);
    half_t* dy = dv.alloc<half_t>((size_t)B * hw * Cpad);
    launch_mbstd(dx, B, hw, C, Cpad, batch_size, group, 1e-8f, dy, 0);
    int rc = finish();
    if (rc) return rc;
    return down16(out, dy, (size_t)B * hw * Cpad);
}

extern "C" int glass_op_resize(int32_t device, int32_t B, int32_t R, int32_t S, int32_t ps, const float* y, float* patches) {
    OPREQ(y && patches && S % ps == 0, "bad argument");
    GLASS_HIP(hipSetDevice(device));
    Dev dv;
    float* dy = dv.up32(y, (size_t)B * 3 * R * R);
    const size_t n = (size_t)B * 3 * S * S;
    half_t* dp = dv.alloc<half_t>(n);
    launch_resize_patches(dy, B, R, S, ps, 3 * ps * ps, dp, 0);
    int rc = finish();
    if (rc) return rc;
    return down16(patches, dp, n);
}

extern "C" int glass_op_preprocess(int32_t device, int32_t B, int32_t R, int32_t S, int32_t ps, int32_t resize_mode, int32_t normalize,
                                   const float* y, float* patches) {
    OPREQ(y && patches && B > 0 && R > 0 && ps > 0 && S > 0 && S % ps == 0, "bad argument");
    if (int rc = glass_clip_preprocess_supported(R, S, resize_mode, normalize)) return rc;
    ResizeTaps t;
    std::string why;
    if (resize_mode) OPREQ(build_resize_taps(R, S, resize_mode, t, why), why);
    GLASS_HIP(hipSetDevice(device));
    Dev dv;
    float* dy = dv.up32(y, (size_t)B * 3 * R * R);
    const size_t n = (size_t)B * 3 * S * S;
    half_t* dp = dv.alloc<half_t>(n);
    OPREQ(dy && dp, "device allocation failed");
    if (resize_mode == 0 && normalize == 0) {
        launch_resize_patches(dy, B, R, S, ps, 3 * ps * ps, dp, 0);
    } else {
        ResizeTapsDev td;
        if (resize_mode) {
            float* dt = dv.up32(t.table.data(), t.table.size());
            OPREQ(dt, "device allocation failed");
            td.table = dt; td.n4 = (int)(t.table.size() / 4); td.ts = t.ts; td.lds_bytes = t.lds_bytes;
        }
        launch_preprocess_patches(dy, B, R, S, ps, 3 * ps * ps, resize_mode, normalize, td, dp, 0);
    }
    int rc = finish();
    if (rc) return rc;
    return down16(patches, dp, n);
}

extern "C" int glass_op_layernorm(int32_t device, int32_t M, int32_t D, const float* x, const float* g, const float* b, float* out) {
    OPREQ(x && g && b && out, "null argument");
    GLASS_HIP(hipSetDevice(device));
    Dev dv;
    float* dx = dv.up32(x, (size_t)M * D); float* dg = dv.up32(g, D); float* db = dv.up32(b, D);
    float* dout = dv.alloc<float>((size_t)M * D);
    launch_layernorm(dx, D, M, D, dg, db, nullptr, dout, 0);
    int rc = finish();
    if (rc) return rc;
    GLASS_HIP(hipMemcpy(out, dout, (size_t)M * D * sizeof(float), hipMemcpyDeviceToHost));
    return GLASS_OK;
}

extern "C" int glass_op_attention(int32_t device, int32_t n_img, int32_t L, int32_t heads, int32_t causal,
                                  const float* qkv, float* out) {
    OPREQ(qkv && out && n_img > 0 && heads > 0 && L >= 1 && L <= 4096, "bad argument (1 <= L <= 4096)");
    GLASS_HIP(hipSetDevice(device));
    Dev dv;
    const int D = heads * 64;
    half_t* dq = dv.up16(qkv, (size_t)n_img * L * 3 * D);
    half_t* dout = dv.alloc<half_t>((size_t)n_img * L * D);
    launch_attention(dq, n_img, L, heads, 64, causal, dout, 0);
    int rc = finish();
    if (rc) return rc;
    return down16(out, dout, (size_t)n_img * L * D);
}

extern "C" int glass_op_noise(int32_t device, int32_t n_mb, int32_t hw, uint32_t layer, uint32_t mb0,
                              uint32_t generation, uint64_t seed, float* out) {
    OPREQ(out, "null argument");
    GLASS_HIP(hipSetDevice(device));
    Dev dv;
    float* d = dv.alloc<float>((size_t)n_mb * hw);
    launch_noise(d, n_mb, hw, layer, mb0, generation, seed, 0);
    int rc = finish();
    if (rc) return rc;
    GLASS_HIP(hipMemcpy(out, d, (size_t)n_mb * hw * sizeof(float), hipMemcpyDeviceToHost));
    return GLASS_OK;
}

extern "C" int glass_op_gpt2_sample(int32_t device, int32_t rows, int32_t V, const float* logits, float temperature, int32_t top_k,
                                    uint64_t seed, int32_t generation, int32_t first_row, int32_t step, int32_t purpose, int32_t* out) {
    OPREQ(logits && out && rows > 0 && V > 0, "bad argument");
    OPREQ(temperature > 0.f && temperature < INFINITY, "temperature must be a finite value > 0");
    OPREQ(top_k >= 0 && top_k <= GPT2_SAMPLE_TOPK_MAX, "top_k must lie in [0, 256]");
    OPREQ(gpt2_sample_supported(V), "vocabulary too large for the sampler (> 131072)");
    GLASS_HIP(hipSetDevice(device));
    Dev dv;
    float* d = dv.up32(logits, (size_t)rows * V);
    int* sp = dv.alloc<int>(GPT2_SP_WORDS);
    int* o = dv.alloc<int>(rows);
    OPREQ(d && sp && o, "hipMalloc failed");
    int32_t h[GPT2_SP_WORDS];
    h[GPT2_SP_SEED_LO] = (int32_t)(uint32_t)(seed & 0xFFFFFFFFu);
    h[GPT2_SP_SEED_HI] = (int32_t)(uint32_t)(seed >> 32);
    h[GPT2_SP_GEN] = generation;
    h[GPT2_SP_ROW0] = first_row;
    h[GPT2_SP_PURPOSE] = purpose;
    memcpy(&h[GPT2_SP_TEMP], &temperature, sizeof(float));
    h[GPT2_SP_TOPK] = top_k;
    h[GPT2_SP_STEP] = step;
    GLASS_HIP(hipMemcpy(sp, h, sizeof h, hipMemcpyHostToDevice));
    launch_gpt2_sample(d, rows, V, sp, o, nullptr, 0);
    int rc = finish();
    if (rc) return rc;
    GLASS_HIP(hipMemcpy(out, o, (size_t)rows * sizeof(int), hipMemcpyDeviceToHost));
    return GLASS_OK;
}

extern "C" int glass_op_gpt2_gemm(int32_t device, int32_t form, int32_t M, int32_t N, int32_t K, int32_t lda, int32_t mode, int32_t width,
                                  const float* a, const float* w, const float* bias, const float* lng, const float* lnb, const float* pst_in,
                                  int32_t np_in, float* out, float* stats_out, float* pst_out, int32_t* splits) {
    OPREQ(a && w && out && splits, "null argument");
    OPREQ(form >= 0 && form <= 3 && mode >= 0 && mode <= 2, "form must lie in [0, 3], mode in [0, 2]");
    OPREQ(M > 0 && N > 0 && K > 0 && K % 4 == 0 && lda >= K && lda % 4 == 0 && width > 0, "bad shape (K, lda multiples of 4, lda >= K)");
    OPREQ((lng == nullptr) == (lnb == nullptr), "LayerNorm gain and bias come together");
    OPREQ(!lng || form >= 2, "LayerNorm is fused on the operand of forms 2 and 3 only");
    OPREQ(!lng || mode != 2, "the residual products have no fused LayerNorm");
    const bool ln = lng != nullptr;
    if (form == 2) {
        OPREQ(gemm_f32_step_supported(M, K, lda, ln), "launch_gemm_f32_step does not take this shape (M <= 64, K % 64 == 0, K <= 1024 with LayerNorm)");
        OPREQ(!ln || (lda == K && stats_out), "fused LayerNorm: gpt2_finalize_kernel makes the statistics of dense rows (lda == K), returned in stats_out");
        OPREQ(mode != 2 || (N <= 1024 && stats_out), "a residual product is finished by gpt2_finalize_kernel: N <= 1024, statistics returned in stats_out");
    }
    if (form == 3) {
        OPREQ(gemm_f32_rowblk_supported(M, N, K, lda, ln, pst_out != nullptr),
              "launch_gemm_f32_rowblk does not take this shape (M <= 64, N % 32 == 0, K % 768 == 0, K <= 1024 with LayerNorm, N <= 768 with statistics)");
        OPREQ(ln == (pst_in != nullptr), "fused LayerNorm consumes the row partials pst_in [M, np_in, 2]");
        OPREQ(!ln || (np_in >= 1 && np_in <= 24 && K % np_in == 0), "np_in must divide K and lie in [1, 24]");
    }
    GLASS_HIP(hipSetDevice(device));
    Dev dv;
    const size_t part_elems = (size_t)16 * M * 4 * width;
    float* da = dv.up32(a, (size_t)M * lda); float* dw = dv.up32(w, (size_t)N * K); float* db = dv.up32(bias, N);
    float* dg = dv.up32(lng, K); float* dlb = dv.up32(lnb, K);
    const size_t rows_alloc = (size_t)(M + 63) / 64 * 64, n_guard = (rows_alloc - M) * N;
    float* dout = dv.alloc<float>(rows_alloc * N);
    float* part = dv.alloc<float>(part_elems);
    float* dstats = dv.alloc<float>((size_t)M * 2);
    float* dpi = ln && form == 3 ? dv.up32(pst_in, (size_t)M * np_in * 2) : nullptr;
    float* dpo = pst_out ? dv.alloc<float>((size_t)M * (N / 32 + 1) * 2) : nullptr;
    OPREQ(da && dw && dout && part && dstats && (!bias || db) && (!ln || (dg && dlb)) && (!pst_out || dpo), "hipMalloc failed");
    GLASS_HIP(hipMemset(dout, 0xff, rows_alloc * N * sizeof(float)));
    if (mode == 2) GLASS_HIP(hipMemcpy(dout, out, (size_t)M * N * sizeof(float), hipMemcpyHostToDevice));
    int S = 1;
    if (form == 0 || form == 1) {
        launch_gemm_f32(da, dw, db, dout, M, N, K, lda, N, mode, 0, part, part_elems, form == 0);
    } else if (form == 2) {
        if (ln) launch_gpt2_finalize(nullptr, 0, nullptr, da, M, K, dstats, 0);
        S = launch_gemm_f32_step(da, dw, db, dout, M, N, K, lda, N, mode, 0, part, part_elems, ln ? dstats : nullptr, dg, dlb);
        OPREQ(S > 0, "launch_gemm_f32_step refused the shape");
        if (mode == 2) launch_gpt2_finalize(S > 1 ? part : nullptr, S, db, dout, M, N, dstats, 0);
        else if (S > 1) launch_gpt2_reduce(part, S, db, dout, M, N, N, mode, 0);
    } else {
        OPREQ(launch_gemm_f32_rowblk(da, dw, db, dout, M, N, K, lda, N, mode, 0, dpi, np_in, dg, dlb, dpo), "launch_gemm_f32_rowblk refused the shape");
    }
    int rc = finish();
    if (rc) return rc;
    *splits = S;
    GLASS_HIP(hipMemcpy(out, dout, (size_t)M * N * sizeof(float), hipMemcpyDeviceToHost));
    std::vector<uint32_t> guard(n_guard);
    GLASS_HIP(hipMemcpy(guard.data(), dout + (size_t)M * N, n_guard * sizeof(float), hipMemcpyDeviceToHost));
    for (size_t i = 0; i < n_guard; ++i)
        if (guard[i] != 0xffffffffu) {
            glass_set_error("gpt2_gemm: the product stored to row " + std::to_string(M + i / N) + " >= M");
            return GLASS_ERR_STATE;
        }
    if (stats_out && form == 2 && (ln || mode == 2)) GLASS_HIP(hipMemcpy(stats_out, dstats, (size_t)M * 2 * sizeof(float), hipMemcpyDeviceToHost));
    if (pst_out && form == 3) GLASS_HIP(hipMemcpy(pst_out, dpo, (size_t)M * (N / 32) * 2 * sizeof(float), hipMemcpyDeviceToHost));
    return GLASS_OK;
}

extern "C" int glass_op_gpt2_attention(int32_t device, int32_t form, int32_t P, int32_t nd, int32_t past, int32_t Tmax, int32_t heads, int32_t S,
                                       const float* qkv, const float* bias, float* kc, float* vc, float* out) {
    OPREQ(qkv && kc && vc && out, "null argument");
    OPREQ(form >= 0 && form <= 2, "form must lie in [0, 2]");
    OPREQ(P > 0 && heads > 0 && nd > 0 && past >= 0 && past + nd <= Tmax, "bad shape (past + nd <= Tmax)");
    const int D = heads * 64;
    if (form == 2) {
        OPREQ(nd == 1 && Tmax <= 64, "gpt2_attention_step_kernel: one new position, Tmax <= 64");
        OPREQ(S >= 0 && S <= 16, "S must lie in [0, 16] (0: finished qkv values)");
    } else {
        OPREQ(S == 0 && !bias, "the general kernel takes finished qkv values");
        const int ns = form == 1 ? Tmax : past + nd;
        OPREQ(gpt2_attention_lds_bytes(nd, ns) <= GPT2_ATTENTION_LDS_MAX,
              "gpt2_attention_kernel: nd * 65 + 2 * ns * 65 + nd * (ns + 1) floats exceed 160 KB of LDS");
    }
    GLASS_HIP(hipSetDevice(device));
    Dev dv;
    const size_t nq = (size_t)(form == 2 && S > 0 ? S : 1) * P * nd * 3 * D, nc = (size_t)P * Tmax * D, no = (size_t)P * nd * D;
    float* dq = dv.up32(qkv, nq); float* db = dv.up32(bias, 3 * D);
    float* dk = dv.up32(kc, nc); float* dvc = dv.up32(vc, nc);
    float* dout = dv.alloc<float>(no);
    int* dpast = dv.alloc<int>(3);
    OPREQ(dq && dk && dvc && dout && dpast && (!bias || db), "hipMalloc failed");
    const int state[3] = {past, 1, 0};
    GLASS_HIP(hipMemcpy(dpast, state, sizeof state, hipMemcpyHostToDevice));
    GLASS_HIP(hipMemset(dout, 0xff, no * sizeof(float)));
    if (form == 2) launch_gpt2_attention_step(dq, S > 0 ? dq : nullptr, S > 0 ? S : 1, db, dk, dvc, P, Tmax, heads, dout, 0, dpast);
    else launch_gpt2_attention(dq, dk, dvc, P, nd, form == 1 ? 0 : past, Tmax, heads, dout, 0, form == 1 ? dpast : nullptr);
    int rc = finish();
    if (rc) return rc;
    GLASS_HIP(hipMemcpy(out, dout, no * sizeof(float), hipMemcpyDeviceToHost));
    GLASS_HIP(hipMemcpy(kc, dk, nc * sizeof(float), hipMemcpyDeviceToHost));
    GLASS_HIP(hipMemcpy(vc, dvc, nc * sizeof(float), hipMemcpyDeviceToHost));
    return GLASS_OK;
// ... 125 lines not shown
```

### clip_glass_amd/ops.py

```python
import ctypes as C

import numpy as np

from .engine import _check, _f32, _fp, load_library


class ConvDesc(C.Structure):
    _fields_ = [("B", C.c_int32), ("H", C.c_int32), ("W", C.c_int32), ("Cin", C.c_int32), ("Cout", C.c_int32),
                ("KS", C.c_int32), ("stride", C.c_int32), ("pad", C.c_int32), ("up", C.c_int32),
                ("Ho", C.c_int32), ("Wo", C.c_int32), ("broadcast_x", C.c_int32), ("act", C.c_int32),
                ("batch_size", C.c_int32), ("impl", C.c_int32),
                ("noise_strength", C.c_float), ("out_scale", C.c_float),
                ("x", C.POINTER(C.c_float)), ("w", C.POINTER(C.c_float)), ("sn", C.POINTER(C.c_float)),
                ("dscale", C.POINTER(C.c_float)), ("noise", C.POINTER(C.c_float)), ("bias", C.POINTER(C.c_float)),
                ("res", C.POINTER(C.c_float)), ("y", C.POINTER(C.c_float)),
                ("trgb_w", C.POINTER(C.c_float)), ("trgb_b", C.POINTER(C.c_float)), ("trgb_sn", C.POINTER(C.c_float)),
                ("trgb_smax", C.POINTER(C.c_float)), ("trgb_yprev", C.POINTER(C.c_float)),
                ("trgb_yout", C.POINTER(C.c_float)),
                ("skip_x", C.POINTER(C.c_float)), ("skip_w", C.POINTER(C.c_float)), ("xs_out", C.POINTER(C.c_float)),
                ("x_planar8", C.c_int32), ("x_planar32", C.c_int32)]


def to_planar8(a):
    B, H, W, Cc = a.shape
# ... 57 lines not shown
            a, p = _opt(val)
            keep.append(a)
            setattr(d, name, p)
    if xs_out is not None:
        d.xs_out = _fp(xs_out)
    yrgb = None
    if torgb is not None:
        yrgb = np.empty((B, 3, Ho, Wo), dtype=np.float32)
        for name in ("w", "b", "sn", "smax", "yprev"):
            a, p = _opt(torgb.get(name))
            keep.append(a)
            if p is not None:
                setattr(d, "trgb_" + name, p)
        d.trgb_yout = _fp(yrgb)
    lib.glass_op_conv.argtypes = [C.c_int32, C.POINTER(ConvDesc)]
    _check(lib, lib.glass_op_conv(device, C.byref(d)))
    if both:
        return yrgb, y
    return yrgb if yrgb is not None else y


def gemm(a, w, bias=None, mode=3, impl=0, acc=None, device=0):
    lib = load_library()
    a = _f32(a); w = _f32(w)
    M, K = a.shape
    N = w.shape[0]
    out = _f32(acc).copy() if acc is not None else np.empty((M, N), dtype=np.float32)
    b, bp = _opt(bias)
    lib.glass_op_gemm.argtypes = [C.c_int32] * 4 + [C.POINTER(C.c_float)] * 3 + [C.c_int32, C.c_int32, C.POINTER(C.c_float)]
    _check(lib, lib.glass_op_gemm(device, M, N, K, _fp(a), _fp(w), bp, mode, impl, _fp(out)))
    return out


def dense(x, wt, bias=None, in_sq=False, mode=0, eps_row=None, device=0):
    lib = load_library()
    x = _f32(x); wt = _f32(wt)
    P, K = x.shape
    N = wt.shape[1]
    out = np.empty((P, N), dtype=np.float32)
    b, bp = _opt(bias)
    e, ep = _opt(eps_row)
    fp = C.POINTER(C.c_float)
    lib.glass_op_dense.argtypes = [C.c_int32] * 4 + [fp, fp, fp, C.c_int32, C.c_int32, fp, fp]
    _check(lib, lib.glass_op_dense(device, P, K, N, _fp(x), _fp(wt), bp, int(in_sq), mode, ep, _fp(out)))
    return out


def torgb(x, wrgb, bias, sn, smax, yprev=None, device=0):
    lib = load_library()
    x = _f32(x)
    B, H, _, Cc = x.shape
    wrgb, bias, sn, smax = _f32(wrgb), _f32(bias), _f32(sn), _f32(smax)
    yp, ypp = _opt(yprev)
    out = np.empty((B, 3, H, H), dtype=np.float32)
    fp = C.POINTER(C.c_float)
    lib.glass_op_torgb.argtypes = [C.c_int32] * 4 + [fp] * 7
    _check(lib, lib.glass_op_torgb(device, B, H, Cc, _fp(x), _fp(wrgb), _fp(bias), _fp(sn), _fp(smax), ypp, _fp(out)))
    return out


def blur(x, mode, device=0):
    lib = load_library()
    x = _f32(x)
    B, H, _, Cc = x.shape
    Ho = H + 1 if mode != 1 else H // 2
    out = np.empty((B, Ho, Ho, Cc), dtype=np.float32)
    fp = C.POINTER(C.c_float)
    lib.glass_op_blur.argtypes = [C.c_int32] * 5 + [fp, fp]
    _check(lib, lib.glass_op_blur(device, mode, B, H, Cc, _fp(x), _fp(out)))
    return from_planar32(out, B, Ho, Ho, Cc) if mode == 2 else out


def dblock_down(h, x, w1, wskip, b1, device=0):
    lib = load_library()
    h, x, w1, wskip, b1 = _f32(h), _f32(x), _f32(w1), _f32(wskip), _f32(b1)
    B, R, _, Cin = h.shape
    Cout = w1.shape[0]
    out = np.empty((B, R // 2, R // 2, Cout), dtype=np.float32)
    fp = C.POINTER(C.c_float)
    lib.glass_op_dblock_down.argtypes = [C.c_int32] * 5 + [fp] * 6
    _check(lib, lib.glass_op_dblock_down(device, B, R, Cin, Cout, _fp(h), _fp(x), _fp(w1), _fp(wskip), _fp(b1), _fp(out)))
    return out


def dblock0(y, frgb_w, frgb_b, w0, b0, w1, wskip, b1, impl=0, device=0):
    lib = load_library()
    y, frgb_w, frgb_b, w0, b0, w1, wskip, b1 = (_f32(a) for a in (y, frgb_w, frgb_b, w0, b0, w1, wskip, b1))
    B, _, R, _ = y.shape
    out = np.empty((B, R // 2, R // 2, 64), dtype=np.float32)
    fp = C.POINTER(C.c_float)
    lib.glass_op_dblock0.argtypes = [C.c_int32] * 4 + [fp] * 9
    _check(lib, lib.glass_op_dblock0(device, B, R, impl, _fp(y), _fp(frgb_w), _fp(frgb_b), _fp(w0), _fp(b0), _fp(w1), _fp(wskip),
                                     _fp(b1), _fp(out)))
    return from_planar8(out, B, R // 2, R // 2, 64) if impl == 2 else out


def fromrgb(y, w, bias, device=0):
    lib = load_library()
    y, w, bias = _f32(y), _f32(w), _f32(bias)
    B, _, R, _ = y.shape
    Cout = w.shape[0]
    out = np.empty((B, R, R, Cout), dtype=np.float32)
    fp = C.POINTER(C.c_float)
    lib.glass_op_fromrgb.argtypes = [C.c_int32] * 4 + [fp] * 4
    _check(lib, lib.glass_op_fromrgb(device, B, R, Cout, _fp(y), _fp(w), _fp(bias), _fp(out)))
    return out


def mbstd(x, Cpad, batch_size, group=4, device=0):
    lib = load_library()
    x = _f32(x)
    B, hw, Cc = x.shape
    out = np.empty((B, hw, Cpad), dtype=np.float32)
    fp = C.POINTER(C.c_float)
    lib.glass_op_mbstd.argtypes = [C.c_int32] * 7 + [fp, fp]
    _check(lib, lib.glass_op_mbstd(device, B, hw, Cc, Cpad, batch_size, group, _fp(x), _fp(out)))
    return out


def resize(y, S, ps, device=0):
    lib = load_library()
    y = _f32(y)
    B, _, R, _ = y.shape
    G = S // ps
    out = np.empty((B * G * G, 3 * ps * ps), dtype=np.float32)
    fp = C.POINTER(C.c_float)
    lib.glass_op_resize.argtypes = [C.c_int32] * 5 + [fp, fp]
    _check(lib, lib.glass_op_resize(device, B, R, S, ps, _fp(y), _fp(out)))
    return out


def preprocess(y, S, ps, resize_mode=0, normalize=0, device=0):
    lib = load_library()
    y = _f32(y)
    B, _, R, _ = y.shape
    G = S // ps
    out = np.empty((B * G * G, 3 * ps * ps), dtype=np.float32)
    fp = C.POINTER(C.c_float)
    lib.glass_op_preprocess.argtypes = [C.c_int32] * 7 + [fp, fp]
    _check(lib, lib.glass_op_preprocess(device, B, R, S, ps, int(resize_mode), int(normalize), _fp(y), _fp(out)))
    return out


def layernorm(x, g, b, device=0):
    lib = load_library()
    x, g, b = _f32(x), _f32(g), _f32(b)
    out = np.empty_like(x)
    fp = C.POINTER(C.c_float)
    lib.glass_op_layernorm.argtypes = [C.c_int32] * 3 + [fp] * 4
    _check(lib, lib.glass_op_layernorm(device, x.shape[0], x.shape[1], _fp(x), _fp(g), _fp(b), _fp(out)))
    return out


def attention(qkv, n_img, L, heads, causal=False, device=0):
    lib = load_library()
    qkv = _f32(qkv)
    out = np.empty((n_img * L, heads * 64), dtype=np.float32)
    fp = C.POINTER(C.c_float)
    lib.glass_op_attention.argtypes = [C.c_int32] * 5 + [fp, fp]
    _check(lib, lib.glass_op_attention(device, n_img, L, heads, int(causal), _fp(qkv), _fp(out)))
    return out


def noise(n_mb, hw, layer, mb0, generation, seed, device=0):
    lib = load_library()
    out = np.empty((n_mb, hw), dtype=np.float32)
    lib.glass_op_noise.argtypes = [C.c_int32, C.c_int32, C.c_int32, C.c_uint32, C.c_uint32, C.c_uint32, C.c_uint64,
                                   C.POINTER(C.c_float)]
    _check(lib, lib.glass_op_noise(device, n_mb, hw, layer, mb0, generation, seed, _fp(out)))
    return out


def gpt2_sample(logits, temperature, top_k, seed, generation, first_row, step, purpose=0, device=0):
    lib = load_library()
    lg = _f32(logits)
    rows, V = lg.shape
    out = np.empty(rows, dtype=np.int32)
    ip = C.POINTER(C.c_int32)
    lib.glass_op_gpt2_sample.argtypes = [C.c_int32, C.c_int32, C.c_int32, C.POINTER(C.c_float), C.c_float, C.c_int32, C.c_uint64,
                                         C.c_int32, C.c_int32, C.c_int32, C.c_int32, ip]
    _check(lib, lib.glass_op_gpt2_sample(device, rows, V, _fp(lg), float(temperature), int(top_k), int(seed) & 0xFFFFFFFFFFFFFFFF,
                                         int(generation), int(first_row), int(step), int(purpose), out.ctypes.data_as(ip)))
    return out


GPT2_GEMM_FORMS = {"prefill": 0, "decode": 1, "step": 2, "rowblk": 3}


def gpt2_gemm(a, w, bias=None, mode=0, form="step", res=None, ln=None, pst_in=None, want_pst=False, width=None, device=0):
    lib = load_library()
    a = np.asarray(a, dtype=np.float32)
    assert a.ndim == 2 and a.strides[1] == 4 and a.strides[0] % 4 == 0
    M, K = a.shape
    lda = a.strides[0] // 4 if M > 1 else K
    abuf = np.zeros((M, lda), dtype=np.float32)
    abuf[:, :K] = a
    if lda > K:
        abuf[:, K:] = np.nan
    w = _f32(w)
    N = w.shape[0]
    assert w.shape == (N, K)
    f = GPT2_GEMM_FORMS[form]
    out = np.empty((M, N), dtype=np.float32)
    if mode == 2:
        out[...] = res
    fp, ip = C.POINTER(C.c_float), C.POINTER(C.c_int32)
    bias_a, bias_p = _opt(bias)
    g_a, g_p = _opt(None if ln is None else ln[0])
    b_a, b_p = _opt(None if ln is None else ln[1])
    pi_a, pi_p = _opt(pst_in)
    np_in = 0 if pst_in is None else int(pi_a.shape[1])
    stats = np.full((M, 2), np.nan, dtype=np.float32)
    pst = np.full((M, max(N // 32, 1), 2), np.nan, dtype=np.float32) if want_pst else None
    S = C.c_int32(0)
    lib.glass_op_gpt2_gemm.argtypes = [C.c_int32] * 8 + [fp] * 6 + [C.c_int32, fp, fp, fp, ip]
    _check(lib, lib.glass_op_gpt2_gemm(device, f, M, N, K, lda, int(mode), int(width or min(N, K)), _fp(abuf), _fp(w), bias_p, g_p, b_p, pi_p,
                                       np_in, _fp(out), _fp(stats), None if pst is None else _fp(pst), C.byref(S)))
    return dict(out=out, S=int(S.value), stats=stats, pst=pst)


def gpt2_attention(qkv, kc, vc, past, heads, form="general", bias=None, device=0):
    lib = load_library()
    kc, vc = np.array(kc, dtype=np.float32, order="C"), np.array(vc, dtype=np.float32, order="C")
    P, Tmax, D = kc.shape
    assert vc.shape == kc.shape and D == heads * 64
    qkv = _f32(qkv)
    f = {"general": 0, "general_dev": 1, "step": 2}[form]
    if qkv.ndim == 3:
        S, nd = qkv.shape[0], 1
        assert f == 2 and qkv.shape[1:] == (P, 3 * D)
    else:
        S, nd = 0, qkv.shape[0] // P
        assert qkv.shape == (P * nd, 3 * D)
    out = np.empty((P * nd, D), dtype=np.float32)
    fp = C.POINTER(C.c_float)
    bias_a, bias_p = _opt(bias)
    lib.glass_op_gpt2_attention.argtypes = [C.c_int32] * 8 + [fp] * 5
    _check(lib, lib.glass_op_gpt2_attention(device, f, P, nd, int(past), Tmax, heads, S, _fp(qkv), bias_p, _fp(kc), _fp(vc), _fp(out)))
    return out, kc, vc


def gpt2_head(x, wte, lng, lnb, tail=False, wpe=None, past=0, step=0, device=0):
    lib = load_library()
    x, wte, lng, lnb = _f32(x), _f32(wte), _f32(lng), _f32(lnb)
    M, K = x.shape
    V = wte.shape[0]
    NB = (V + 31) // 32
    fp, ip = C.POINTER(C.c_float), C.POINTER(C.c_int32)
    token = np.full(M, -1, dtype=np.int32)
    stats = np.full((M, 2), np.nan, dtype=np.float32)
    lib.glass_op_gpt2_head.argtypes = [C.c_int32] * 5 + [fp] * 5 + [C.c_int32] * 3 + [fp, fp, ip, ip, fp, fp, fp, ip]
    if not tail:
        logits = np.empty((M, V), dtype=np.float32)
        pv = np.empty((M, NB), dtype=np.float32)
        pi = np.empty((M, NB), dtype=np.int32)
        _check(lib, lib.glass_op_gpt2_head(device, M, V, K, 0, _fp(x), _fp(wte), _fp(lng), _fp(lnb), None, 0, 0, 0, _fp(logits), _fp(pv),
                                           pi.ctypes.data_as(ip), token.ctypes.data_as(ip), _fp(stats), None, None, None))
        return dict(logits=logits, pair_val=pv, pair_idx=pi, token=token, stats=stats)
    wpe = _f32(wpe)
    x_next = np.full((M, K), np.nan, dtype=np.float32)
    stats_next = np.full((M, 2), np.nan, dtype=np.float32)
    state = np.full(3, -1, dtype=np.int32)
    _check(lib, lib.glass_op_gpt2_head(device, M, V, K, 1, _fp(x), _fp(wte), _fp(lng), _fp(lnb), _fp(wpe), wpe.shape[0], int(past), int(step),
                                       None, None, None, token.ctypes.data_as(ip), _fp(stats), _fp(x_next), _fp(stats_next),
                                       state.ctypes.data_as(ip)))
    return dict(token=token, stats=stats, x_next=x_next, stats_next=stats_next, state=state)


def gpt2_embed_step(token, wte, wpe, past, step, device=0):
    lib = load_library()
    wte, wpe = _f32(wte), _f32(wpe)
    tok = np.ascontiguousarray(token, dtype=np.int32)
    M, (V, K) = tok.shape[0], wte.shape
    x = np.full((M, K), np.nan, dtype=np.float32)
    stats = np.full((M, 2), np.nan, dtype=np.float32)
    fp, ip = C.POINTER(C.c_float), C.POINTER(C.c_int32)
    lib.glass_op_gpt2_embed_step.argtypes = [C.c_int32] * 4 + [ip, fp, fp] + [C.c_int32] * 3 + [fp, fp]
    _check(lib, lib.glass_op_gpt2_embed_step(device, M, V, K, tok.ctypes.data_as(ip), _fp(wte), _fp(wpe), wpe.shape[0], int(past), int(step),
                                             _fp(x), _fp(stats)))
    return x, stats


def mfma_probe(a, b, device=0):
    lib = load_library()
    a, b = _f32(a), _f32(b)
    d = np.empty((32, 32), dtype=np.float32)
    fp = C.POINTER(C.c_float)
    lib.glass_op_mfma_probe.argtypes = [C.c_int32, fp, fp, fp]
    _check(lib, lib.glass_op_mfma_probe(device, _fp(a), _fp(b), _fp(d)))
    return d


def host_pack_conv(w, up=False):
    lib = load_library()
    w = _f32(w)
    Cout, Cin, KS, _ = w.shape
    out = np.empty((KS * KS, (4 if up else 1) * Cout, Cin), dtype=np.float32)
    fp = C.POINTER(C.c_float)
    lib.glass_host_pack_conv.argtypes = [fp, C.c_int32, C.c_int32, C.c_int32, C.c_int32, fp]
    _check(lib, lib.glass_host_pack_conv(_fp(w), Cout, Cin, KS, int(up), _fp(out)))
    return out


RESIZE_MAX_TAPS = 32


# ... 9 lines not shown
```

### include/glass_ops.h

```cpp
#ifndef GLASS_OPS_H
#define GLASS_OPS_H
#include <stdint.h>
#ifdef __cplusplus
extern "C" {
#endif

typedef struct glass_conv_desc {
    int32_t B, H, W, Cin, Cout;
    int32_t KS, stride, pad;
    int32_t up;
    int32_t Ho, Wo;
    int32_t broadcast_x;
    int32_t act;
    int32_t batch_size;
    int32_t impl;
    float noise_strength, out_scale;
    const float* x;
    const float* w;
    const float* sn;
    const float* dscale;
    const float* noise;
    const float* bias;
    const float* res;
    float* y;
    const float* trgb_w;
    const float* trgb_b;
    const float* trgb_sn;
    const float* trgb_smax;
    const float* trgb_yprev;
    float* trgb_yout;
    const float* skip_x;
    const float* skip_w;
    float* xs_out;
    int32_t x_planar8;
    int32_t x_planar32;
} glass_conv_desc;

int glass_op_conv(int32_t device, const glass_conv_desc* d);
int glass_op_gemm(int32_t device, int32_t M, int32_t N, int32_t K, const float* a, const float* w,
                  const float* bias, int32_t mode, int32_t impl, float* out);
int glass_op_dense(int32_t device, int32_t P, int32_t K, int32_t N, const float* x, const float* wt ,
                   const float* bias, int32_t in_sq, int32_t mode, const float* eps_row, float* out);
int glass_op_torgb(int32_t device, int32_t B, int32_t H, int32_t C, const float* x, const float* wrgb ,
                   const float* bias, const float* sn, const float* smax, const float* yprev, float* yout);
int glass_op_blur(int32_t device, int32_t mode , int32_t B, int32_t H, int32_t C,
                  const float* x, float* out);
int glass_op_dblock_down(int32_t device, int32_t B, int32_t R, int32_t Cin, int32_t Cout, const float* h, const float* x,
                         const float* w1, const float* wskip, const float* b1, float* y);
int glass_op_dblock0(int32_t device, int32_t B, int32_t R, int32_t impl, const float* y, const float* frgb_w, const float* frgb_b,
                     const float* w0, const float* b0, const float* w1, const float* wskip, const float* b1, float* out);
int glass_op_fromrgb(int32_t device, int32_t B, int32_t R, int32_t Cout, const float* y ,
                     const float* w , const float* bias, float* out );
int glass_op_mbstd(int32_t device, int32_t B, int32_t hw, int32_t C, int32_t Cpad, int32_t batch_size, int32_t group,
                   const float* x, float* out);
int glass_op_resize(int32_t device, int32_t B, int32_t R, int32_t S, int32_t ps, const float* y ,
                    float* patches );
int glass_op_preprocess(int32_t device, int32_t B, int32_t R, int32_t S, int32_t ps, int32_t resize_mode, int32_t normalize,
                        const float* y , float* patches );
int glass_op_layernorm(int32_t device, int32_t M, int32_t D, const float* x, const float* g, const float* b, float* out);
int glass_op_attention(int32_t device, int32_t n_img, int32_t L, int32_t heads, int32_t causal, const float* qkv,
                       float* out);
int glass_op_noise(int32_t device, int32_t n_mb, int32_t hw, uint32_t layer, uint32_t mb0, uint32_t generation,
                   uint64_t seed, float* out);
int glass_op_gpt2_sample(int32_t device, int32_t rows, int32_t V, const float* logits, float temperature, int32_t top_k,
                         uint64_t seed, int32_t generation, int32_t first_row, int32_t step, int32_t purpose, int32_t* out);
int glass_op_gpt2_gemm(int32_t device, int32_t form, int32_t M, int32_t N, int32_t K, int32_t lda, int32_t mode, int32_t width,
                       const float* a, const float* w, const float* bias, const float* lng, const float* lnb, const float* pst_in,
                       int32_t np_in, float* out, float* stats_out, float* pst_out, int32_t* splits);
int glass_op_gpt2_attention(int32_t device, int32_t form, int32_t P, int32_t nd, int32_t past, int32_t Tmax, int32_t heads, int32_t S,
                            const float* qkv, const float* bias, float* kc, float* vc, float* out);
int glass_op_gpt2_head(int32_t device, int32_t M, int32_t V, int32_t K, int32_t tail, const float* x, const float* wte, const float* lng,
                       const float* lnb, const float* wpe, int32_t npos, int32_t past, int32_t step, float* logits, float* pair_val,
                       int32_t* pair_idx, int32_t* token, float* stats, float* x_next, float* stats_next, int32_t* state);
int glass_op_gpt2_embed_step(int32_t device, int32_t M, int32_t V, int32_t K, const int32_t* token, const float* wte, const float* wpe,
                             int32_t npos, int32_t past, int32_t step, float* x, float* stats);
int glass_op_mfma_probe(int32_t device, const float* a , const float* b , float* d );

int glass_host_pack_conv(const float* w, int32_t Cout, int32_t Cin, int32_t KS, int32_t up, float* out);
int glass_host_resize_taps(int32_t R, int32_t S, int32_t mode, int32_t* start, int32_t* count, float* taps, int32_t max);

#ifdef __cplusplus
}
#endif
#endif
```

Baseline: 2257 candidates/s.

## Fuse CLIP LayerNorms into GEMM prologue/epilogue and fuse CLIP head

Removes the standalone LayerNorm kernels in the CLIP transformer blocks. The residual-add GEMM epilogue now writes per-tile partial mean/M2 row statistics. The following QKV/FC GEMM merges those statistics and normalizes the fp32 residual stream while staging its A tile to LDS. This drops the f16 ln16 intermediate buffer and two launches per block. The final head (LayerNorm, projection, cosine) also becomes a single kernel. The cost is fp32 A-operand loads in place of f16, extra epilogue reductions and syncs, and a hard failure if the tiled GEMM refuses a shape.

After: 2224 candidates/s. -1.4%, worse.

```diff
diff --git a/clip_glass_amd/csrc/clip.cpp b/clip_glass_amd/csrc/clip.cpp
--- a/clip_glass_amd/csrc/clip.cpp
+++ b/clip_glass_amd/csrc/clip.cpp
@@ -158,7 +158,7 @@
     return GLASS_OK;
 }
 
-static void run_blocks(glass_engine* e, const std::vector<ClipBlock>& blk, int l0, int l1, float* x, half_t* ln16, half_t* qkv, half_t* att,
+static void run_blocks(glass_engine* e, const std::vector<ClipBlock>& blk, int l0, int l1, float* x, float* stats, half_t* qkv, half_t* att,
                        half_t* hid, int T, int seqs, int W, int heads, int causal, hipStream_t st, const char* pfx) {
     const int M = seqs * T;
     char buf[48];
@@ -169,24 +169,37 @@
     };
     auto gemm = [&](const GemmParams& g, const char* op) {
         if (pfx) run_gemm(e, g, tag(op));
-        else if (!launch_gemm_tiled(g, st)) launch_gemm_direct(g, st);
-    };
-    auto layernorm = [&](const float* g, const float* b) {
-        Prof pr(e, tag("layernorm"), 0, 6.0 * M * W);
-        launch_layernorm(x, W, M, W, g, b, ln16, nullptr, st);
-    };
+        else if (!launch_gemm_tiled(g, st) && e->launch_error.empty()) e->launch_error = std::string("gemm_tiled refuses the LayerNorm-fused product ") + op;
+    };
+    auto ln_gemm = [&](const float* g, const float* b, int np, const half_t* w, int N, const float* bias, int mode, half_t* out, const char* op) {
+        GemmParams q = gemm_params(nullptr, w, M, N, W, bias, mode, out, nullptr, T);
+        q.a32 = x; q.ln_stats = stats; q.ln_np = np; q.ln_pw = np ? W / np : 0; q.ln_g = g; q.ln_b = b; q.ln_eps = 1e-5f;
+        gemm(q, op);
+    };
+    auto res_params = [&](const half_t* a, const half_t* w, int K, const float* bias) {
+        GemmParams q = gemm_params(a, w, M, W, K, bias, 2, nullptr, x, T);
+        q.stats_out = stats;
+        return q;
+    };
+    auto n_partials = [&](const GemmParams& q) {
+        const int bn = gemm_tiled_bn(q);
+        return bn ? W / bn : 0;
+    };
+    int np = l0 == 0 ? W / 64 : n_partials(res_params(hid, blk[l0 - 1].w_proj, 4 * W, nullptr));
     for (int li = l0; li < l1; ++li) {
         const ClipBlock& b = blk[li];
-        layernorm(b.ln1_g, b.ln1_b);
-        gemm(gemm_params(ln16, b.w_qkv, M, 3 * W, W, b.b_qkv, 0, qkv, nullptr, T), "qkv");
+        ln_gemm(b.ln1_g, b.ln1_b, np, b.w_qkv, 3 * W, b.b_qkv, 0, qkv, "qkv");
         {
             Prof pr(e, tag("attention"), 4.0 * seqs * heads * (double)T * T * 64, 8.0 * M * W);
             launch_attention(qkv, seqs, T, heads, 64, causal, att, st);
         }
-        gemm(gemm_params(att, b.w_out, M, W, W, b.b_out, 2, nullptr, x, T), "attn_out");
-        layernorm(b.ln2_g, b.ln2_b);
-        gemm(gemm_params(ln16, b.w_fc, M, 4 * W, W, b.b_fc, 1, hid, nullptr, T), "mlp_fc");
-        gemm(gemm_params(hid, b.w_proj, M, W, 4 * W, b.b_proj, 2, nullptr, x, T), "mlp_proj");
+        GemmParams q = res_params(att, b.w_out, W, b.b_out);
+        np = n_partials(q);
+        gemm(q, "attn_out");
+        ln_gemm(b.ln2_g, b.ln2_b, np, b.w_fc, 4 * W, b.b_fc, 1, hid, "mlp_fc");
+        q = res_params(hid, b.w_proj, 4 * W, b.b_proj);
+        np = n_partials(q);
+        gemm(q, "mlp_proj");
     }
 }
 
@@ -195,21 +208,19 @@
     const int W = c.clip_width, G = c.clip_res / c.clip_patch, T = G * G + 1;
     run_gemm(e, gemm_params(e->d_patches, e->c_patch_w, P * G * G, W, clip_patch_k(c), nullptr, 3, nullptr, e->d_pe, G * G), "clip.patch_embed");
     Prof pr(e, "clip.embed_lnpre", 0, 8.0 * P * T * W);
-    launch_embed_lnpre(e->d_pe, e->c_cls, e->c_pos, e->c_lnpre_g, e->c_lnpre_b, P, T, W, e->d_x, e->cur);
+    launch_embed_lnpre(e->d_pe, e->c_cls, e->c_pos, e->c_lnpre_g, e->c_lnpre_b, P, T, W, e->d_x, e->d_lnstats, e->cur);
 }
 void run_clip_layers(glass_engine* e, int P, int l0, int l1) {
     const glass_config& c = e->cfg;
     const int G = c.clip_res / c.clip_patch;
-    run_blocks(e, e->cblk, l0, std::min(l1, (int)e->cblk.size()), e->d_x, e->d_ln16, e->d_qkv, e->d_attn, e->d_hid, G * G + 1, P, c.clip_width, c.clip_heads, 0, e->cur, "clip");
+    run_blocks(e, e->cblk, l0, std::min(l1, (int)e->cblk.size()), e->d_x, e->d_lnstats, e->d_qkv, e->d_attn, e->d_hid, G * G + 1, P, c.clip_width, c.clip_heads, 0, e->cur, "clip");
 }
 void run_clip_head(glass_engine* e, int P) {
     const glass_config& c = e->cfg;
     const int W = c.clip_width, G = c.clip_res / c.clip_patch, T = G * G + 1;
     Prof pr(e, "clip.head", 2.0 * P * W * c.clip_embed, 4.0 * W * c.clip_embed);
-    launch_layernorm(e->d_x, (long long)T * W, P, W, e->c_lnpost_g, e->c_lnpost_b, nullptr, e->d_cls, e->cur);
-    launch_dense(e->d_cls, W, P, W, e->c_proj, c.clip_embed, nullptr, e->d_feat, c.clip_embed, 0, 0, nullptr, 0,
-                 e->cur);
-    launch_cosine(e->d_feat, e->d_target, P, c.clip_embed, e->d_sim, e->cur);
+    launch_clip_head(e->d_x, (long long)T * W, P, W, e->c_lnpost_g, e->c_lnpost_b, e->c_proj, c.clip_embed, e->d_target, e->d_feat, e->d_sim,
+                     e->cur);
 }
 void run_clip(glass_engine* e, int P) {
     run_clip_embed(e, P);
@@ -261,7 +272,7 @@
         if (err == hipSuccess) err = owned_alloc(tw.owned, &tw.x, (size_t)M * W);
         if (err == hipSuccess) err = owned_alloc(tw.owned, &tw.cls, (size_t)n_texts * W);
         if (err == hipSuccess) err = owned_alloc(tw.owned, &tw.feat, (size_t)n_texts * E);
-        if (err == hipSuccess) err = owned_alloc(tw.owned, &tw.ln16, (size_t)M * W);
+        if (err == hipSuccess) err = owned_alloc(tw.owned, &tw.lnstats, (size_t)M * (W / 64) * 2);
         if (err == hipSuccess) err = owned_alloc(tw.owned, &tw.qkv, (size_t)M * 3 * W);
         if (err == hipSuccess) err = owned_alloc(tw.owned, &tw.att, (size_t)M * W);
         if (err == hipSuccess) err = owned_alloc(tw.owned, &tw.hid, (size_t)M * 4 * W);
@@ -276,8 +287,8 @@
     hipStream_t st = e->stream;
     hipMemcpyAsync(tw.d_tok, tokens, (size_t)M * sizeof(int), hipMemcpyHostToDevice, st);
     hipMemcpyAsync(tw.d_rows, eot.data(), (size_t)n_texts * sizeof(int), hipMemcpyHostToDevice, st);
-    launch_embed_text(tw.d_tok, e->t_tok, e->t_pos, M, ctx, W, tw.x, st);
-    run_blocks(e, e->tblk, 0, (int)e->tblk.size(), tw.x, tw.ln16, tw.qkv, tw.att, tw.hid, ctx, n_texts, W, heads, 1, st, nullptr);
+    launch_embed_text(tw.d_tok, e->t_tok, e->t_pos, M, ctx, W, tw.x, tw.lnstats, st);
+    run_blocks(e, e->tblk, 0, (int)e->tblk.size(), tw.x, tw.lnstats, tw.qkv, tw.att, tw.hid, ctx, n_texts, W, heads, 1, st, nullptr);
     launch_layernorm_rows(tw.x, tw.d_rows, n_texts, W, e->t_lnf_g, e->t_lnf_b, tw.cls, st);
     launch_dense(tw.cls, W, n_texts, W, e->t_proj, E, nullptr, tw.feat, E, 0, 0, nullptr, 0, st);
     err = hipMemcpyAsync(out_feat, tw.feat, (size_t)n_texts * E * sizeof(float), hipMemcpyDeviceToHost, st);
diff --git a/clip_glass_amd/csrc/common.h b/clip_glass_amd/csrc/common.h
--- a/clip_glass_amd/csrc/common.h
+++ b/clip_glass_amd/csrc/common.h
@@ -194,4 +194,18 @@
     int g_on, g_h, g_w, g_hc, g_wc, g_stride, g_pad, g_ks, g_cin;
     long long g_xbs;
     int ld;
+    float* stats_out;
+    const float* a32;
+    const float* ln_stats;
+    int ln_np, ln_pw;
+    const float *ln_g, *ln_b;
+    float ln_eps;
 };
+__device__ __forceinline__ void ln_merge_partials(const float* st, int np, int pw, float eps, float& mean, float& rstd) {
+    float sm = 0.f, sq = 0.f;
+    for (int i = 0; i < np; ++i) { sm += st[2 * i]; sq += st[2 * i + 1]; }
+    mean = sm / (float)np;
+    float so = 0.f;
+    for (int i = 0; i < np; ++i) { const float d = st[2 * i] - mean; so += d * d; }
+    rstd = rsqrtf((sq + (float)pw * so) / (float)(np * pw) + eps);
+}
diff --git a/clip_glass_amd/csrc/engine.cpp b/clip_glass_amd/csrc/engine.cpp
--- a/clip_glass_amd/csrc/engine.cpp
+++ b/clip_glass_amd/csrc/engine.cpp
@@ -500,11 +500,10 @@
     if (Kp != (size_t)3 * ps * ps) GLASS_HIP(hipMemset(e->d_patches, 0, (size_t)P * G * G * Kp * sizeof(half_t)));
     if ((rc = dev_alloc(e, &e->d_pe, (size_t)P * G * G * W))) return rc;
     if ((rc = dev_alloc(e, &e->d_x, (size_t)P * T * W))) return rc;
-    if ((rc = dev_alloc(e, &e->d_ln16, (size_t)P * T * W))) return rc;
+    if ((rc = dev_alloc(e, &e->d_lnstats, (size_t)P * T * (W / 64) * 2))) return rc;
     if ((rc = dev_alloc(e, &e->d_qkv, (size_t)P * T * 3 * W))) return rc;
     if ((rc = dev_alloc(e, &e->d_attn, (size_t)P * T * W))) return rc;
     if ((rc = dev_alloc(e, &e->d_hid, (size_t)P * T * 4 * W))) return rc;
-    if ((rc = dev_alloc(e, &e->d_cls, (size_t)P * W))) return rc;
     if ((rc = dev_alloc(e, &e->d_feat, (size_t)P * c.clip_embed))) return rc;
     if ((rc = dev_alloc(e, &e->d_sim, (size_t)P))) return rc;
     if ((rc = dev_alloc(e, &e->d_dis, (size_t)P))) return rc;
@@ -617,8 +616,13 @@
     pr.ran(tag, k);
 }
 void run_gemm(glass_engine* e, const GemmParams& p, const char* tag) {
-    Prof pr(e, tag, 2.0 * p.M * p.N * p.K, 2.0 * ((double)p.M * p.K + (double)p.N * p.K + (double)p.M * p.N));
+    Prof pr(e, tag, 2.0 * p.M * p.N * p.K,
+            2.0 * ((double)p.M * p.K + (double)p.N * p.K + (double)p.M * p.N) + (p.a32 ? 2.0 * p.M * p.K + 8.0 * p.M * p.ln_np : 0.0));
     const char* k = launch_gemm_tiled(p, e->cur);
+    if (!k && (p.a32 || p.stats_out)) {
+        if (e->launch_error.empty()) e->launch_error = std::string("gemm_tiled refuses the LayerNorm-fused product ") + tag;
+        k = "(refused)";
+    }
     if (!k) k = launch_gemm_direct(p, e->cur);
     pr.ran(tag, k);
 }
diff --git a/clip_glass_amd/csrc/engine.h b/clip_glass_amd/csrc/engine.h
--- a/clip_glass_amd/csrc/engine.h
+++ b/clip_glass_amd/csrc/engine.h
@@ -146,8 +146,8 @@
     struct TextWork {
         int n_texts = 0;
         int *d_tok = nullptr, *d_rows = nullptr;
-        float *x = nullptr, *cls = nullptr, *feat = nullptr;
-        half_t *ln16 = nullptr, *qkv = nullptr, *att = nullptr, *hid = nullptr;
+        float *x = nullptr, *cls = nullptr, *feat = nullptr, *lnstats = nullptr;
+        half_t *qkv = nullptr, *att = nullptr, *hid = nullptr;
         std::vector<void*> owned;
     } twork;
     int t_width = 0, t_ctx = 0, t_vocab = 0;
@@ -171,8 +171,9 @@
     size_t act_elems = 0;
     float* ybuf[4] = {nullptr, nullptr, nullptr, nullptr};
     float* d_img = nullptr;
-    half_t *d_patches = nullptr, *d_ln16 = nullptr, *d_qkv = nullptr, *d_attn = nullptr, *d_hid = nullptr;
-    float *d_pe = nullptr, *d_x = nullptr, *d_cls = nullptr, *d_feat = nullptr, *d_sim = nullptr, *d_dis = nullptr,
+    half_t *d_patches = nullptr, *d_qkv = nullptr, *d_attn = nullptr, *d_hid = nullptr;
+    float* d_lnstats = nullptr;
+    float *d_pe = nullptr, *d_x = nullptr, *d_feat = nullptr, *d_sim = nullptr, *d_dis = nullptr,
           *d_F = nullptr, *d_dh = nullptr, *d_dh_part = nullptr;
     half_t* d_dfin = nullptr;
     float* h_pinned = nullptr;
diff --git a/clip_glass_amd/csrc/gemm_tiled.hip b/clip_glass_amd/csrc/gemm_tiled.hip
--- a/clip_glass_amd/csrc/gemm_tiled.hip
+++ b/clip_glass_amd/csrc/gemm_tiled.hip
@@ -4,7 +4,7 @@
 
 #define GROWB 144
 
-template <int BN, bool GATHER = false>
+template <int BN, bool GATHER = false, bool LNA = false>
 __global__ __launch_bounds__(256, 2) void gemm_tiled_kernel(GemmParams p) {
     if (p.batch > 1) {
         p.a += (long long)blockIdx.z * p.a_bs;
@@ -29,6 +29,8 @@
     const int part = t & 7;
 
     h8 ra[NA], rb[NB];
+    f4 rx[NA][2], rg[2], rsh[2];
+    float lmean[NA], lrstd[NA];
     long long gbase[GATHER ? NA : 1];
     int giy[GATHER ? NA : 1], gix[GATHER ? NA : 1], okm = 0;
     if (GATHER) {
@@ -53,6 +55,18 @@
                 ra[k] = *(const h8*)(p.a + (ok ? gbase[k] + toff : (long long)part * 8));
                 okm |= (ok ? 1 : 0) << k;
             }
+        } else if (LNA) {
+#pragma unroll
+            for (int k = 0; k < NA; ++k) {
+                const float* src = p.a32 + (long long)min(m0 + (t >> 3) + 32 * k, p.M - 1) * p.K + k0 + part * 8;
+                rx[k][0] = *(const f4*)src;
+                rx[k][1] = *(const f4*)(src + 4);
+            }
+#pragma unroll
+            for (int h = 0; h < 2; ++h) {
+                rg[h] = *(const f4*)(p.ln_g + k0 + part * 8 + 4 * h);
+                rsh[h] = *(const f4*)(p.ln_b + k0 + part * 8 + 4 * h);
+            }
         } else {
 #pragma unroll
         for (int k = 0; k < NA; ++k) {
@@ -70,8 +84,22 @@
     };
     auto store = [&]() {
         const h8 zero = {0, 0, 0, 0, 0, 0, 0, 0};
+        if (LNA) {
+#pragma unroll
+            for (int k = 0; k < NA; ++k) {
+                h8 o;
+#pragma unroll
+                for (int h = 0; h < 2; ++h) {
+                    const f4 v = (rx[k][h] - lmean[k]) * lrstd[k] * rg[h] + rsh[h];
+#pragma unroll
+                    for (int q = 0; q < 4; ++q) o[4 * h + q] = (half_t)v[q];
+                }
+                *(h8*)(As + ((t >> 3) + 32 * k) * GROWB + part * 16) = m0 + (t >> 3) + 32 * k < p.M ? o : zero;
+            }
+        } else {
 #pragma unroll
         for (int k = 0; k < NA; ++k) *(h8*)(As + ((t >> 3) + 32 * k) * GROWB + part * 16) = (!GATHER || ((okm >> k) & 1)) ? ra[k] : zero;
+        }
 #pragma unroll
         for (int k = 0; k < NB; ++k) *(h8*)(Bs + ((t >> 3) + 32 * k) * GROWB + part * 16) = rb[k];
     };
@@ -85,6 +113,22 @@
             for (int q = 0; q < 16; ++q) acc[i][j][q] = 0.f;
 
     load(0);
+    if (LNA) {
+        float* sst = (float*)smem;
+        if (t < 128) {
+            float mean, rstd;
+            ln_merge_partials(p.ln_stats + (long long)min(m0 + t, p.M - 1) * p.ln_np * 2, p.ln_np, p.ln_pw, p.ln_eps, mean, rstd);
+            sst[2 * t] = mean;
+            sst[2 * t + 1] = rstd;
+        }
+        __syncthreads();
+#pragma unroll
+        for (int k = 0; k < NA; ++k) {
+            lmean[k] = sst[2 * ((t >> 3) + 32 * k)];
+            lrstd[k] = sst[2 * ((t >> 3) + 32 * k) + 1];
+        }
+        __syncthreads();
+    }
     for (int k0 = 0; k0 < p.K; k0 += 64) {
         if (k0 > 0) __syncthreads();
         store();
@@ -105,6 +149,9 @@
                 for (int j = 0; j < NJ; ++j) acc[i][j] = mfma32(wf[j], xf[i], acc[i][j]);
         }
     }
+    const bool st_on = p.mode == 2 && p.stats_out != nullptr;
+    float* sst = (float*)smem;
+    if (st_on) __syncthreads();
     f4 bq[NJ][4];
 #pragma unroll
     for (int j = 0; j < NJ; ++j)
@@ -146,6 +193,10 @@
                     if (p.mode == 2) {
 #pragma unroll
                         for (int q = 0; q < 4; ++q) o[q] = rq[j][g][q] + v[q];
+                        if (st_on) {
+#pragma unroll
+                            for (int q = 0; q < 4; ++q) acc[i][j][g * 4 + q] = o[q];
+                        }
                     } else {
 #pragma unroll
                         for (int q = 0; q < 4; ++q) o[q] = p.mode == 4 ? lrelu_sqrt2(v[q]) : v[q];
@@ -154,31 +205,77 @@
                 }
             }
         }
+        if (st_on) {
+            float s = 0.f;
+#pragma unroll
+            for (int j = 0; j < NJ; ++j)
+#pragma unroll
+                for (int r = 0; r < 16; ++r) s += acc[i][j][r];
+            s += __shfl_xor(s, 32);
+            const float mean = s * (2.f / BN);
+            float qq = 0.f;
+#pragma unroll
+            for (int j = 0; j < NJ; ++j)
+#pragma unroll
+                for (int r = 0; r < 16; ++r) { const float d = acc[i][j][r] - mean; qq += d * d; }
+            qq += __shfl_xor(qq, 32);
+            if (kh == 0) {
+                sst[(wn * 128 + wm * 64 + i * 32 + lr) * 2] = mean;
+                sst[(wn * 128 + wm * 64 + i * 32 + lr) * 2 + 1] = qq;
+            }
+        }
+    }
+    if (st_on) {
+        __syncthreads();
+        if (t < 128 && m0 + t < p.M) {
+            const float a0 = sst[2 * t], a1 = sst[2 * (128 + t)], mean = (a0 + a1) * 0.5f, d0 = a0 - mean, d1 = a1 - mean;
+            const float m2 = (sst[2 * t + 1] + sst[2 * (128 + t) + 1]) + (float)(BN / 2) * (d0 * d0 + d1 * d1);
+            float* so = p.stats_out + ((long long)(m0 + t) * gy + n0 / BN) * 2;
+            so[0] = mean;
+            so[1] = m2;
+        }
     }
 }
 
-const char* launch_gemm_tiled(const GemmParams& p, hipStream_t st) {
-    if (p.K % 64 != 0 || p.ldo % 4 != 0 || (p.M < 64 && !p.kpt) || (p.kpt && p.kpt % 64 != 0)) return nullptr;
-    const unsigned gx = (unsigned)((p.M + 127) / 128), gz = p.batch > 1 ? p.batch : 1;
+int gemm_tiled_bn(const GemmParams& p) {
+    if (p.K % 64 != 0 || p.ldo % 4 != 0 || (p.M < 64 && !p.kpt && !p.a32 && !p.stats_out) || (p.kpt && p.kpt % 64 != 0)) return 0;
+    const long long gx = (p.M + 127) / 128, gz = p.batch > 1 ? p.batch : 1;
     const long long gx_n = p.cand_rows ? ((long long)p.cand_rows * GLASS_NOMINAL_POP + 127) / 128 : gx;
     const long long gz_n = p.cand_batch ? GLASS_NOMINAL_POP : gz;
     const bool fills = gx_n * (p.N / 128) * gz_n >= 256;
-    if (p.g_on && (!p.kpt || p.kpt != p.g_cin || p.g_cin % 64 != 0)) return nullptr;
-    if (p.N % 128 == 0 && fills) {
+    if (p.g_on && (!p.kpt || p.kpt != p.g_cin || p.g_cin % 64 != 0)) return 0;
+    const bool plain = !p.g_on && !p.kpt && !p.ld && p.batch <= 1;
+    if (p.stats_out && !(plain && p.mode == 2)) return 0;
+    if (p.a32 && !(plain && p.ln_stats && p.ln_g && p.ln_b && p.ln_np > 0 && (long long)p.ln_np * p.ln_pw == p.K)) return 0;
+    if (p.N % 128 == 0 && fills) return 128;
+    return p.N % 64 == 0 ? 64 : 0;
+}
+
+const char* launch_gemm_tiled(const GemmParams& p, hipStream_t st) {
+    const int bn = gemm_tiled_bn(p);
+    if (!bn) return nullptr;
+    const unsigned gx = (unsigned)((p.M + 127) / 128), gz = p.batch > 1 ? p.batch : 1;
+    const dim3 grid(8 * ((gx * (p.N / bn) + 7) / 8), 1, gz);
+    if (bn == 128) {
+        if (p.a32) {
+            hipLaunchKernelGGL((gemm_tiled_kernel<128, false, true>), grid, dim3(256), 0, st, p);
+            return "gemm_tiled_kernel<128,false,true>";
+        }
         if (p.g_on) {
-            hipLaunchKernelGGL((gemm_tiled_kernel<128, true>), dim3(8 * ((gx * (p.N / 128) + 7) / 8), 1, gz), dim3(256), 0, st, p);
+            hipLaunchKernelGGL((gemm_tiled_kernel<128, true>), grid, dim3(256), 0, st, p);
             return "gemm_tiled_kernel<128,true>";
         }
-        hipLaunchKernelGGL(gemm_tiled_kernel<128>, dim3(8 * ((gx * (p.N / 128) + 7) / 8), 1, gz), dim3(256), 0, st, p);
+        hipLaunchKernelGGL(gemm_tiled_kernel<128>, grid, dim3(256), 0, st, p);
         return "gemm_tiled_kernel<128>";
     }
-    if (p.N % 64 == 0) {
-        if (p.g_on) {
-            hipLaunchKernelGGL((gemm_tiled_kernel<64, true>), dim3(8 * ((gx * (p.N / 64) + 7) / 8), 1, gz), dim3(256), 0, st, p);
-            return "gemm_tiled_kernel<64,true>";
-        }
-        hipLaunchKernelGGL(gemm_tiled_kernel<64>, dim3(8 * ((gx * (p.N / 64) + 7) / 8), 1, gz), dim3(256), 0, st, p);
-        return "gemm_tiled_kernel<64>";
-    }
-    return nullptr;
+    if (p.a32) {
+        hipLaunchKernelGGL((gemm_tiled_kernel<64, false, true>), grid, dim3(256), 0, st, p);
+        return "gemm_tiled_kernel<64,false,true>";
+    }
+    if (p.g_on) {
+        hipLaunchKernelGGL((gemm_tiled_kernel<64, true>), grid, dim3(256), 0, st, p);
+        return "gemm_tiled_kernel<64,true>";
+    }
+    hipLaunchKernelGGL(gemm_tiled_kernel<64>, grid, dim3(256), 0, st, p);
+    return "gemm_tiled_kernel<64>";
 }
diff --git a/clip_glass_amd/csrc/kernels.h b/clip_glass_amd/csrc/kernels.h
--- a/clip_glass_amd/csrc/kernels.h
+++ b/clip_glass_amd/csrc/kernels.h
@@ -8,6 +8,7 @@
 const char* launch_gemm_direct(const GemmParams& p, hipStream_t st);
 const char* launch_conv_tiled(const ConvParams& p, hipStream_t st);
 const char* launch_gemm_tiled(const GemmParams& p, hipStream_t st);
+int gemm_tiled_bn(const GemmParams& p);
 const char* launch_conv_stream(const ConvParams& p, hipStream_t st);
 const char* launch_conv_gemm(const ConvParams& p, half_t* ws_a, long long cap_a, float* ws_c, long long cap_c, hipStream_t st);
 bool conv_stream_applies(const ConvParams& p);
@@ -82,15 +83,18 @@
                   half_t* out, hipStream_t st);
 
 void launch_embed_lnpre(const float* patch_emb, const float* cls, const float* pos, const float* g,
-                        const float* b, int P, int T, int D, float* x, hipStream_t st);
-void launch_embed_text(const int* tokens, const float* tok_emb, const float* pos, int n_rows, int ctx, int D, float* x,
+                        const float* b, int P, int T, int D, float* x, float* stats, hipStream_t st);
+void launch_embed_text(const int* tokens, const float* tok_emb, const float* pos, int n_rows, int ctx, int D, float* x, float* stats,
                        hipStream_t st);
+void launch_row_partials(const float* x, int M, int D, float* stats, hipStream_t st);
 void launch_layernorm(const float* x, long long row_stride, int M, int D, const float* g, const float* b,
                       half_t* out16, float* out32, hipStream_t st);
 void launch_layernorm_rows(const float* x, const int* rows, int M, int D, const float* g, const float* b, float* out32, hipStream_t st);
 void launch_attention(const half_t* qkv, int n_img, int L, int heads, int hd, int causal, half_t* out,
                       hipStream_t st);
 void launch_cosine(const float* feat, const float* target, int P, int D, float* sim, hipStream_t st);
+void launch_clip_head(const float* x, long long row_stride, int P, int D, const float* g, const float* b, const float* proj, int E,
+                      const float* target, float* feat, float* sim, hipStream_t st);
 void launch_assemble_F(const float* sim, const float* dis, int P, int n_obj, float* F, hipStream_t st);
 
 void launch_bg_cond(const float* x, int P, int L, int zd, int nc, const float* et, float* cond, hipStream_t st);
diff --git a/clip_glass_amd/csrc/kernels_clip.hip b/clip_glass_amd/csrc/kernels_clip.hip
--- a/clip_glass_amd/csrc/kernels_clip.hip
+++ b/clip_glass_amd/csrc/kernels_clip.hip
@@ -47,31 +47,54 @@
     }
 }
 
+template <typename ValF>
+__device__ __forceinline__ void row_partials64(ValF val, int D, float* st) {
+    const int lane = threadIdx.x & 63;
+    for (int i = 0; i < D / 64; ++i) {
+        const float v = val(64 * i + lane);
+        const float mean = wsum(v) * (1.f / 64.f), d = v - mean;
+        const float m2 = wsum(d * d);
+        if (lane == 0) { st[2 * i] = mean; st[2 * i + 1] = m2; }
+    }
+}
+__global__ __launch_bounds__(256) void row_partials_kernel(const float* x, int M, int D, float* stats) {
+    const int row = blockIdx.x * 4 + (threadIdx.x >> 6);
+    if (row >= M) return;
+    const float* xr = x + (long long)row * D;
+    row_partials64([&](int i) { return xr[i]; }, D, stats + (long long)row * (D / 64) * 2);
+}
+void launch_row_partials(const float* x, int M, int D, float* stats, hipStream_t st) {
+    hipLaunchKernelGGL(row_partials_kernel, dim3((M + 3) / 4), dim3(256), 0, st, x, M, D, stats);
+}
+
 __global__ __launch_bounds__(256) void embed_lnpre_kernel(const float* pe, const float* cls, const float* pos,
                                                           const float* g, const float* b, int P, int T, int D,
-                                                          float* x) {
+                                                          float* x, float* stats) {
     const int row = blockIdx.x * 4 + (threadIdx.x >> 6);
     if (row >= P * T) return;
     const int p = row / T, t = row - p * T;
     const float* src = t == 0 ? cls : pe + ((long long)p * (T - 1) + (t - 1)) * D;
     const float* ps = pos + (long long)t * D;
-    ln_row([&](int i) { return src[i] + ps[i]; }, D, g, b, nullptr, x + (long long)row * D);
+    float* xr = x + (long long)row * D;
+    ln_row([&](int i) { return src[i] + ps[i]; }, D, g, b, nullptr, xr);
+    if (stats) row_partials64([&](int i) { return xr[i]; }, D, stats + (long long)row * (D / 64) * 2);
 }
 void launch_embed_lnpre(const float* patch_emb, const float* cls, const float* pos, const float* g,
-                        const float* b, int P, int T, int D, float* x, hipStream_t st) {
+                        const float* b, int P, int T, int D, float* x, float* stats, hipStream_t st) {
     hipLaunchKernelGGL(embed_lnpre_kernel, dim3((P * T + 3) / 4), dim3(256), 0, st, patch_emb, cls, pos, g, b, P,
-                       T, D, x);
-}
-
-__global__ void embed_text_kernel(const int* tokens, const float* tok_emb, const float* pos, int ctx, int D, float* x) {
+                       T, D, x, stats);
+}
+
+__global__ void embed_text_kernel(const int* tokens, const float* tok_emb, const float* pos, int ctx, int D, float* x, float* stats) {
     const int row = blockIdx.x;
     const float* te = tok_emb + (long long)tokens[row] * D;
     const float* pe = pos + (long long)(row % ctx) * D;
     for (int i = threadIdx.x; i < D; i += blockDim.x) x[(long long)row * D + i] = te[i] + pe[i];
-}
-void launch_embed_text(const int* tokens, const float* tok_emb, const float* pos, int n_rows, int ctx, int D, float* x,
+    if (stats && threadIdx.x < 64) row_partials64([&](int i) { return te[i] + pe[i]; }, D, stats + (long long)row * (D / 64) * 2);
+}
+void launch_embed_text(const int* tokens, const float* tok_emb, const float* pos, int n_rows, int ctx, int D, float* x, float* stats,
                        hipStream_t st) {
-    hipLaunchKernelGGL(embed_text_kernel, dim3(n_rows), dim3(128), 0, st, tokens, tok_emb, pos, ctx, D, x);
+    hipLaunchKernelGGL(embed_text_kernel, dim3(n_rows), dim3(128), 0, st, tokens, tok_emb, pos, ctx, D, x, stats);
 }
 
 __global__ __launch_bounds__(256) void layernorm_kernel(const float* x, long long row_stride, int M, int D,
@@ -387,6 +410,47 @@
     hipLaunchKernelGGL(cosine_kernel, dim3(P), dim3(64), 0, st, feat, target, D, sim);
 }
 
+__global__ __launch_bounds__(1024) void clip_head_kernel(const float* x, long long row_stride, int D, const float* g, const float* b,
+                                                         const float* proj, int E, const float* target, float* feat, float* sim) {
+    extern __shared__ float head_s[];
+    float* cls = head_s;
+    float* fs = head_s + D;
+    const int p = blockIdx.x, t = threadIdx.x;
+    const float* xr = x + (long long)p * row_stride;
+    if (t < 64) ln_row([&](int i) { return xr[i]; }, D, g, b, nullptr, cls);
+    __syncthreads();
+    for (int n = t; n < E; n += blockDim.x) {
+        float acc = 0.f;
+        int k = 0;
+        for (; k + 16 <= D; k += 16) {
+            float w[16];
+#pragma unroll
+            for (int u = 0; u < 16; ++u) w[u] = proj[(long long)(k + u) * E + n];
+#pragma unroll
+            for (int u = 0; u < 16; ++u) acc = __builtin_fmaf(w[u], cls[k + u], acc);
+        }
+        for (; k < D; ++k) acc = __builtin_fmaf(proj[(long long)k * E + n], cls[k], acc);
+        acc += 0.f;
+        fs[n] = acc;
+        feat[(long long)p * E + n] = acc;
+    }
+    __syncthreads();
+    if (t >= 64) return;
+    float xy = 0.f, xx = 0.f, yy = 0.f;
+    for (int i = t; i < E; i += 64) {
+        const float a = fs[i], c = target[i];
+        xy += a * c; xx += a * a; yy += c * c;
+    }
+    xy = wsum(xy); xx = wsum(xx); yy = wsum(yy);
+    if (t == 0) sim[p] = xy / fmaxf(sqrtf(xx) * sqrtf(yy), 1e-8f);
+}
+void launch_clip_head(const float* x, long long row_stride, int P, int D, const float* g, const float* b, const float* proj, int E,
+                      const float* target, float* feat, float* sim, hipStream_t st) {
+    const int threads = std::min(1024, (E + 63) / 64 * 64);
+    hipLaunchKernelGGL(clip_head_kernel, dim3(P), dim3(threads), (size_t)(D + E) * sizeof(float), st, x, row_stride, D, g, b, proj, E,
+                       target, feat, sim);
+}
+
 __global__ void assemble_F_kernel(const float* sim, const float* dis, int P, int n_obj, float* F) {
     const int p = blockIdx.x * blockDim.x + threadIdx.x;
     if (p >= P) return;
diff --git a/clip_glass_amd/csrc/ops.hip b/clip_glass_amd/csrc/ops.hip
--- a/clip_glass_amd/csrc/ops.hip
+++ b/clip_glass_amd/csrc/ops.hip
@@ -379,6 +379,89 @@
     return GLASS_OK;
 }
 
+extern "C" int glass_op_gemm_ln(int32_t device, int32_t M, int32_t N, int32_t K, int32_t mode, const float* a, float* x, const float* w,
+                                const float* bias, const float* lng, const float* lnb, const float* pst_in, int32_t np_in, float* out,
+                                float* pst_out, int32_t* np_out, int32_t* pw_out) {
+    OPREQ(x && w && M > 0 && (mode == 2 ? a && pst_out && np_out && pw_out : (mode == 0 || mode == 1) && out && lng && lnb), "bad argument");
+    OPREQ(K % 64 == 0 && N % 64 == 0, "N and K must be multiples of 64");
+    OPREQ(mode == 2 || !pst_in || (np_in > 0 && K % np_in == 0), "np_in must divide the width");
+    GLASS_HIP(hipSetDevice(device));
+    Dev dv;
+    const size_t rows_alloc = (size_t)(M + 127) / 128 * 128, n = (size_t)M * N, n_guard = (rows_alloc - M) * N;
+    GemmParams g;
+    memset(&g, 0, sizeof g);
+    g.w = dv.up16(w, (size_t)N * K); g.M = M; g.N = N; g.K = K; g.bias = dv.up32(bias, N); g.mode = mode; g.ldo = N;
+    half_t* o16 = nullptr; float* o32 = nullptr; float* dst = nullptr;
+    size_t st_n = 0, st_guard = 0;
+    if (mode == 2) {
+        g.a = dv.up16(a, (size_t)M * K);
+        o32 = dv.alloc<float>(rows_alloc * N);
+        GLASS_HIP(hipMemcpy(o32, x, n * sizeof(float), hipMemcpyHostToDevice));
+        GLASS_HIP(hipMemset(o32 + n, 0xff, n_guard * sizeof(float)));
+        g.out32 = o32;
+        dst = dv.alloc<float>(rows_alloc * (N / 64) * 2);
+        g.stats_out = dst;
+        const int bn = gemm_tiled_bn(g);
+        OPREQ(bn > 0, "gemm_tiled refuses this residual product");
+        *np_out = N / bn; *pw_out = bn;
+        st_n = (size_t)M * (N / bn) * 2; st_guard = rows_alloc * (N / 64) * 2 - st_n;
+        GLASS_HIP(hipMemset(dst, 0xff, (st_n + st_guard) * sizeof(float)));
+    } else {
+        g.a32 = dv.up32(x, (size_t)M * K);
+        if (pst_in) { g.ln_stats = dv.up32(pst_in, (size_t)M * np_in * 2); g.ln_np = np_in; }
+        else {
+            float* ds = dv.alloc<float>((size_t)M * (K / 64) * 2);
+            launch_row_partials(g.a32, M, K, ds, 0);
+            g.ln_stats = ds; g.ln_np = K / 64;
+        }
+        g.ln_pw = K / g.ln_np; g.ln_g = dv.up32(lng, K); g.ln_b = dv.up32(lnb, K); g.ln_eps = 1e-5f;
+        o16 = dv.alloc<half_t>(rows_alloc * N);
+        GLASS_HIP(hipMemset(o16 + n, 0xff, n_guard * sizeof(half_t)));
+        g.out16 = o16;
+    }
+    if (!launch_gemm_tiled(g, 0)) { glass_set_error("gemm_tiled refuses this LayerNorm-fused product"); return GLASS_ERR_ARG; }
+    int rc = finish();
+    if (rc) return rc;
+    bool touched = false;
+    if (o16) {
+        std::vector<uint16_t> gd(n_guard);
+        GLASS_HIP(hipMemcpy(gd.data(), o16 + n, n_guard * sizeof(half_t), hipMemcpyDeviceToHost));
+        for (uint16_t v : gd) touched |= v != 0xffffu;
+    } else {
+        std::vector<uint32_t> gd(n_guard + st_guard);
+        GLASS_HIP(hipMemcpy(gd.data(), o32 + n, n_guard * sizeof(float), hipMemcpyDeviceToHost));
+        GLASS_HIP(hipMemcpy(gd.data() + n_guard, dst + st_n, st_guard * sizeof(float), hipMemcpyDeviceToHost));
+        for (uint32_t v : gd) touched |= v != 0xffffffffu;
+    }
+    if (touched) { glass_set_error("gemm_tiled stored to a row >= M"); return GLASS_ERR_STATE; }
+    if (o16) return down16(out, o16, n);
+    GLASS_HIP(hipMemcpy(x, o32, n * sizeof(float), hipMemcpyDeviceToHost));
+    GLASS_HIP(hipMemcpy(pst_out, dst, st_n * sizeof(float), hipMemcpyDeviceToHost));
+    return GLASS_OK;
+}
+
+extern "C" int glass_op_clip_head(int32_t device, int32_t P, int32_t T, int32_t W, int32_t E, int32_t impl, const float* x, const float* g,
+                                  const float* b, const float* proj, const float* target, float* feat, float* sim) {
+    OPREQ(x && g && b && proj && target && feat && sim && P > 0 && T > 0 && W > 0 && W <= 4096 && E > 0 && E <= 4096, "bad argument");
+    GLASS_HIP(hipSetDevice(device));
+    Dev dv;
+    float* dx = dv.up32(x, (size_t)P * T * W); float* dg = dv.up32(g, W); float* db = dv.up32(b, W);
+    float* dp = dv.up32(proj, (size_t)W * E); float* dt = dv.up32(target, E);
+    float* dfeat = dv.alloc<float>((size_t)P * E); float* dsim = dv.alloc<float>(P);
+    if (impl == 0) launch_clip_head(dx, (long long)T * W, P, W, dg, db, dp, E, dt, dfeat, dsim, 0);
+    else {
+        float* dcls = dv.alloc<float>((size_t)P * W);
+        launch_layernorm(dx, (long long)T * W, P, W, dg, db, nullptr, dcls, 0);
+        launch_dense(dcls, W, P, W, dp, E, nullptr, dfeat, E, 0, 0, nullptr, 0, 0);
+        launch_cosine(dfeat, dt, P, E, dsim, 0);
+    }
+    int rc = finish();
+    if (rc) return rc;
+    GLASS_HIP(hipMemcpy(feat, dfeat, (size_t)P * E * sizeof(float), hipMemcpyDeviceToHost));
+    GLASS_HIP(hipMemcpy(sim, dsim, (size_t)P * sizeof(float), hipMemcpyDeviceToHost));
+    return GLASS_OK;
+}
+
 extern "C" int glass_op_attention(int32_t device, int32_t n_img, int32_t L, int32_t heads, int32_t causal,
                                   const float* qkv, float* out) {
     OPREQ(qkv && out && n_img > 0 && heads > 0 && L >= 1 && L <= 4096, "bad argument (1 <= L <= 4096)");
diff --git a/clip_glass_amd/ops.py b/clip_glass_amd/ops.py
--- a/clip_glass_amd/ops.py
+++ b/clip_glass_amd/ops.py
@@ -233,6 +233,45 @@
     return out
 
 
+def gemm_ln(x, w, bias=None, mode=0, ln=None, pst_in=None, a=None, device=0):
+    lib = load_library()
+    x = _f32(x).copy(); w = _f32(w)
+    M = x.shape[0]
+    N, K = w.shape
+    fp = C.POINTER(C.c_float)
+    ip = C.POINTER(C.c_int32)
+    lib.glass_op_gemm_ln.argtypes = [C.c_int32] * 5 + [fp] * 7 + [C.c_int32, fp, fp, ip, ip]
+    bb, bp = _opt(bias)
+    np_out, pw_out = C.c_int32(0), C.c_int32(0)
+    if mode == 2:
+        a = _f32(a)
+        assert a.shape == (M, K) and x.shape == (M, N)
+        pst = np.zeros((M, N // 64, 2), dtype=np.float32)
+        _check(lib, lib.glass_op_gemm_ln(device, M, N, K, 2, _fp(a), _fp(x), _fp(w), bp, None, None, None, 0, None, _fp(pst),
+                                         C.byref(np_out), C.byref(pw_out)))
+        return x, pst.reshape(-1)[:M * np_out.value * 2].reshape(M, np_out.value, 2).copy(), pw_out.value
+    assert x.shape == (M, K)
+    g, b = _f32(ln[0]), _f32(ln[1])
+    pi, pip = _opt(pst_in)
+    out = np.empty((M, N), dtype=np.float32)
+    _check(lib, lib.glass_op_gemm_ln(device, M, N, K, mode, None, _fp(x), _fp(w), bp, _fp(g), _fp(b), pip, 0 if pi is None else pi.shape[1],
+                                     _fp(out), None, C.byref(np_out), C.byref(pw_out)))
+    return out
+
+
+def clip_head(x, g, b, proj, target, impl=0, device=0):
+    lib = load_library()
+    x, g, b, proj, target = _f32(x), _f32(g), _f32(b), _f32(proj), _f32(target)
+    P, T, W = x.shape
+    E = proj.shape[1]
+    feat = np.empty((P, E), dtype=np.float32)
+    sim = np.empty(P, dtype=np.float32)
+    fp = C.POINTER(C.c_float)
+    lib.glass_op_clip_head.argtypes = [C.c_int32] * 6 + [fp] * 7
+    _check(lib, lib.glass_op_clip_head(device, P, T, W, E, impl, _fp(x), _fp(g), _fp(b), _fp(proj), _fp(target), _fp(feat), _fp(sim)))
+    return feat, sim
+
+
 def attention(qkv, n_img, L, heads, causal=False, device=0):
     lib = load_library()
     qkv = _f32(qkv)
diff --git a/include/glass_ops.h b/include/glass_ops.h
--- a/include/glass_ops.h
+++ b/include/glass_ops.h
@@ -58,6 +58,11 @@
 int glass_op_preprocess(int32_t device, int32_t B, int32_t R, int32_t S, int32_t ps, int32_t resize_mode, int32_t normalize,
                         const float* y , float* patches );
 int glass_op_layernorm(int32_t device, int32_t M, int32_t D, const float* x, const float* g, const float* b, float* out);
+int glass_op_gemm_ln(int32_t device, int32_t M, int32_t N, int32_t K, int32_t mode, const float* a, float* x, const float* w,
+                     const float* bias, const float* lng, const float* lnb, const float* pst_in, int32_t np_in, float* out,
+                     float* pst_out, int32_t* np_out, int32_t* pw_out);
+int glass_op_clip_head(int32_t device, int32_t P, int32_t T, int32_t W, int32_t E, int32_t impl, const float* x, const float* g,
+                       const float* b, const float* proj, const float* target, float* feat, float* sim);
 int glass_op_attention(int32_t device, int32_t n_img, int32_t L, int32_t heads, int32_t causal, const float* qkv,
                        float* out);
 int glass_op_noise(int32_t device, int32_t n_mb, int32_t hw, uint32_t layer, uint32_t mb0, uint32_t generation,
```
